# L-Scofano/SEEME

Hardware: AMD Instinct MI355X
Metric: sampled seqs/sec (T=196, 50 DDIM steps) (higher is better)
Workload: dtype f32 accumulate (fp16 denoiser weights, fp16 VAE MFMA operands); 1 GPU; config_mld_egobody interactee-only: VAE encode -> 50-step DDIM -> VAE decode, B=32/GPU, T=196, nfeats=132, random-init recipe weights; batch_per_gpu=32, seq_len=196, ddim_steps=50, parallelism=dp1 (independent shards, no collective on the data path)

## Files before the change

### include/seeme_hip.h

```cpp
#ifndef SEEME_HIP_H
#define SEEME_HIP_H

#include <stddef.h>
#include <stdint.h>

#ifdef __cplusplus
extern "C" {
#endif

#define SEEME_D 256
#define SEEME_NLAYERS 5

enum { SEEME_ACT_NONE = 0, SEEME_ACT_RELU = 1, SEEME_ACT_GELU = 2, SEEME_ACT_SILU = 3 };
enum { SEEME_SCHED_NONE = 0, SEEME_SCHED_DDIM = 1, SEEME_SCHED_DDPM = 2 };

int seeme_version(void);
const char* seeme_last_error(void);

#define SEEME_LINEAR_MAX_K 1008
typedef struct {
    const float* A;  int lda;
    const float* A2; int lda2;
    int K1;
    const float* W;  int ldw;
    const float* bias;
    const float* res; int ldr;
    const float* ln_w; const float* ln_b;
    const float* pre_ln_w; const float* pre_ln_b;
    float* Y; int ldy;
    int M, N, K;
    int pre_act;
    int act;
    float eps;
} SeemeLinearArgs;
int seeme_linear(const SeemeLinearArgs* args, void* stream);

typedef struct {
    const float *in_w, *in_b;
    const float *out_w, *out_b;
    const float *l1_w, *l1_b;
    const float *l2_w, *l2_b;
    const float *n1_w, *n1_b, *n2_w, *n2_b;
    const float *ca_in_w, *ca_in_b;
    const float *ca_out_w, *ca_out_b;
    const float *n3_w, *n3_b;
} SeemeXfLayer;

typedef struct {
    SeemeXfLayer layer[SEEME_NLAYERS];
    const float *skip_w[2], *skip_b[2];
    const float *norm_w, *norm_b;
} SeemeSkipStack;

typedef struct { const uint16_t *in_w, *out_w, *l1_w, *l2_w; } SeemeXfLayerH;
typedef struct {
    SeemeXfLayerH enc[SEEME_NLAYERS], dec[SEEME_NLAYERS];
    const uint16_t *enc_skip[2], *dec_skip[2];
    const uint16_t *emb_w, *fin_w, *ca_fold_w;
    const void* dec_pro; int dec_pro_T;
} SeemeVaeWeightsH;

typedef struct {
    int nfeats;
    int ff;
    const float* token;
    const float* pe_enc;
    const float* pe_dec;
    const float* emb_w; int emb_ldw;
    const float* emb_b;
    const float* fin_w;
    const float* fin_b;
    SeemeSkipStack enc, dec;
    const float* ca_fold_w;
    const float* ca_fold_b;
    const SeemeVaeWeightsH* h16;
} SeemeVaeWeights;

size_t seeme_vae_workspace_bytes(int B, int T);

int seeme_vae_encode(const SeemeVaeWeights* w, const float* features, const int32_t* lengths,
                     int B, int T, float* mu, float* logvar, void* workspace, size_t ws_bytes, void* stream);

int seeme_vae_decode(const SeemeVaeWeights* w, const float* z, const int32_t* lengths,
                     int B, int T, float* feats, void* workspace, size_t ws_bytes, void* stream);

size_t seeme_vae_dec_prologue_bytes(int T);
int seeme_vae_dec_prologue_h16(const SeemeVaeWeights* w, int T, void* buf, size_t bytes, void* stream);

typedef struct {
    const void*  wg;   int wdtype;
    const float* vp;
    const int64_t* layout;
    int nhead;
    int ff_sa;
    int ff;
    const float* kv_cat_w; const float* kv_cat_b;
    const float* style_cat_w; const float* style_cat_b;
    const float* time_w1; const float* time_b1; const float* time_w2; const float* time_b2;
    const float* ca_kv_w[SEEME_NLAYERS]; const float* ca_kv_b[SEEME_NLAYERS];
    const float* ca_tn_w[SEEME_NLAYERS]; const float* ca_tn_b[SEEME_NLAYERS];
    const float* ca_fold_w; const float* ca_fold_b;
    const float* ln_ones; const float* ln_zeros;
    int sa_fold;
    const float* ca_pn_w; const float* ca_pn_b;
    const float* ca_po_w; const float* ca_po_b;
} SeemeDenoiserWeights;

#define SEEME_TROW 7680
#define SEEME_CROW 5120

size_t seeme_denoiser_workspace_bytes(int n_rows, int B, int N);

int seeme_denoiser_time_tables(const SeemeDenoiserWeights* w, const float* tfeat, int n_rows,
                               float* ttab, void* workspace, size_t ws_bytes, void* stream);

int seeme_denoiser_cond_tables(const SeemeDenoiserWeights* w, const float* cond, int Bc, int N,
                               float* ctab, void* workspace, size_t ws_bytes, void* stream);

int seeme_denoiser_ca_tables(const SeemeDenoiserWeights* w, const float* ctab, const float* ttab, const int32_t* trow,
                             int trow_per_sample, int n_trow, int Bc, float* catab,
                             void* workspace, size_t ws_bytes, void* stream);

typedef struct {
    int B;
    int N;
    int steps;
    int sched;
    int cfg;
    float guidance_scale;
    const float* latents;
    const float* ctab;
    const float* ttab;
    const int32_t* trow;
    int trow_per_sample;
    const float* coef;
    const float* noise;
    float* out;
    const float* catab;
    float* save;
    int force_query;
    const unsigned char* drop;
    float drop_scale;
    int xcds;
} SeemeSampleArgs;
#define SEEME_DEN_DROP_BYTES 10960

int seeme_denoiser_sample(const SeemeDenoiserWeights* w, const SeemeSampleArgs* a, void* stream);

typedef struct {
    const void*  wgc;  int wdtype;
    const float* vpc;
    int C;
    int placement;
    int flags;
    void* xchg; size_t xchg_bytes;
    int query;
    int samples;
} SeemeDenCluster;
size_t seeme_den_cluster_xchg_bytes(int B, int C);
size_t seeme_den_cluster_ms_xchg_bytes(int B, int C, int samples);
int seeme_den_cluster_layout(int C, int wdtype, int query, int64_t* out, int cap);
int seeme_denoiser_sample_cluster(const SeemeDenoiserWeights* w, const SeemeDenCluster* cl, const SeemeSampleArgs* a, void* stream);

int seeme_den_train_layout(int64_t* out, int cap);
int seeme_den_train_pack(const float* const* mats, float* img_f, float* img_b, const float* const* vec_src,
                         const int* vec_n, const int64_t* vec_dst, int n_vec, float* vp, void* stream);
int seeme_denoiser_backward(const SeemeDenoiserWeights* w, const void* img_bwd, int B, int N, const float* save,
                            const float* ctab, const float* ttab, const int32_t* trow, const float* dout,
                            float* gout, float* dctab, float* dttab, void* stream);
int seeme_denoiser_backward_drop(const SeemeDenoiserWeights* w, const void* img_bwd, int B, int N, const float* save,
                                 const float* ctab, const float* ttab, const int32_t* trow, const float* dout,
                                 float* gout, float* dctab, float* dttab, const unsigned char* drop, float drop_scale, int xcds, void* stream);

int seeme_den_layout(int ff_sa, int ff, int64_t* out, int cap);

typedef struct {
    int V;
    const float* v_template;
    const float* blend_w;
    const float* lbs_weights;
    const float* J_template;
    const float* J_shapedirs;
    const int32_t* parents;
    const float* ex_template;
    const float* ex_shapedirs;
    const float* ex_posedirs;
    const float* ex_weights;
} SeemeSmplModel;

size_t seeme_smpl_workspace_bytes(int M);

int seeme_smpl_lbs(const SeemeSmplModel* m, const float* betas, const float* pose, int pose_is_rotmat,
                   const float* transl, int M, float* joints, float* vertices,
                   void* workspace, size_t ws_bytes, void* stream);

int seeme_smpl_joints_backward(const SeemeSmplModel* m, const float* betas, const float* pose, const float* djoints, int dj_stride,
                               float* dpose, float* dtransl, int M, void* stream);

int seeme_smpl_joints_rot6d(const SeemeSmplModel* m, const float* betas, const float* r6, int order, const float* transl, int M,
                            float* joints, void* stream);
int seeme_smpl_joints_rot6d_backward(const SeemeSmplModel* m, const float* betas, const float* r6, int order, const float* djoints,
                                     int dj_stride, float* dr6, float* dtransl, int M, void* stream);

enum { SEEME_GEO_AA_TO_QUAT = 0, SEEME_GEO_AA_TO_ROTMAT = 1, SEEME_GEO_QUAT_TO_ROTMAT = 2,
       SEEME_GEO_ROT6D_PROHMR = 3, SEEME_GEO_ROT6D_DIFFUSION = 4 };
int seeme_geometry(int op, const float* in, float* out, int M, void* stream);
int seeme_renorm(const float* x, const float* mean, const float* stdv, float* y, long rows, int F, void* stream);

typedef struct {
    int out_dim;
    const float* pos_w; const float* pos_b;
    const float* fc0_w[4]; const float* fc0_b[4];
    const float* fc1_w[4]; const float* fc1_b[4];
    const float* sc_w[4];
    const float* fcc_w; const float* fcc_b;
} SeemePointnetWeights;
size_t seeme_pointnet_workspace_bytes(int B, int P);
int seeme_pointnet_encode(const SeemePointnetWeights* w, const float* points, int B, int P, float* out,
                          void* workspace, size_t ws_bytes, void* stream);

typedef struct {
    const uint16_t* posf;
    const uint16_t* stream[4];
    const uint16_t* sc3f;
} SeemePointnetBf16;
size_t seeme_pointnet_bf16_workspace_bytes(int B, int P);
int seeme_pointnet_encode_bf16(const SeemePointnetWeights* w, const SeemePointnetBf16* wb, const float* points,
                               int B, int P, float* out, void* workspace, size_t ws_bytes, void* stream);

int seeme_den_wgrad(const float* gout, int ldg, int B, const void* tiles, int n_tiles, float* out, void* stream);
int seeme_den_vecgrad(const float* gout, int ldg, int B, const int64_t* idx, int n, float* out, int dx0_col, float* dpe_row0,
                      void* stream);

int seeme_adamw_step(const void* chunks, int n_chunks, void* const* params, const void* const* grads, void* const* exp_avg,
                     void* const* exp_avg_sq, double lr, double beta1, double beta2, double eps, double weight_decay,
                     double step, void* stream);

int seeme_adamw_step_dev(const void* chunks, int n_chunks, void* const* params, const void* const* grads, void* const* exp_avg,
                         void* const* exp_avg_sq, const float* step_lr, double beta1, double beta2, double eps,
                         double weight_decay, void* stream);

typedef struct {
    const void* chunks;
    int n_chunks;
    void* const* params;
    const void* const* grads;
    void* const* exp_avg;
    void* const* exp_avg_sq;
    void* const* ema;
    const float* step_lr;
    double lr, step;
    double beta1, beta2, eps, weight_decay;
    double ema_decay;
    int ema_warmup;
    const float* grad_scale;
} SeemeAdamWEx;
int seeme_adamw_step_ex(const SeemeAdamWEx* a, void* stream);
int seeme_adamw_ex_bytes(void);

size_t seeme_grad_norm_workspace_bytes(int n_chunks);
int seeme_grad_norm(const void* chunks, int n_chunks, const void* const* grads, double max_norm, float* out ,
                    void* ws, size_t ws_bytes, void* stream);

typedef struct {
    int B, N;
    const float* dist;
    int dist_rows;
    const float* eps_z;
    const float* eps_c;
    int slot_c;
    float* cond;
    const float* noise;
    const int64_t* timesteps;
    const float* acp;
    const float* freq;
    int flip_sin_to_cos;
    float* latents;
    float* noisy;
    float* tfeat;
} SeemeGlueRows;
int seeme_glue_rows(const SeemeGlueRows* a, void* stream);
int seeme_glue_ln(const float* x, float* xhat, float* rstd, int M, void* stream);

typedef struct {
    const float* a[10];
    const float* b[10];
    int seg_len[10];
    long a_ks[10];
    long b_ks[10];
    int nseg;
    long a_rs, b_cs;
    float* c;
    long ldc;
    int M, N;
    int a_pro;
    const float* a_p0;
    const float* a_p1;
    int b_pro;
    const float* b_p0;
    const float* b_p1;
    const float* bias;
    int epi;
    const float* e0;
    long e_ld;
    int accumulate;
    float* colsum;
    int tile0, tiles_n;
    int nbatch;
    long a_bstride, b_bstride, c_bstride;
    float alpha;
// ... 178 lines not shown
```

### seeme_amd/_lib.py

```python
from __future__ import annotations

import ctypes as C
import os
from typing import Optional

_HERE = os.path.dirname(os.path.abspath(__file__))
LIB_PATH = os.environ.get("SEEME_HIP_LIB") or os.path.join(_HERE, "libseeme_hip.so")

NLAYERS = 5
TROW = 7680
CROW = 5120
ACT_NONE, ACT_RELU, ACT_GELU, ACT_SILU = 0, 1, 2, 3
SCHED_NONE, SCHED_DDIM, SCHED_DDPM = 0, 1, 2

fp = C.c_void_p


class SeemeError(RuntimeError):
    pass


class LinearArgs(C.Structure):
    _fields_ = [("A", fp), ("lda", C.c_int), ("A2", fp), ("lda2", C.c_int), ("K1", C.c_int),
                ("W", fp), ("ldw", C.c_int), ("bias", fp), ("res", fp), ("ldr", C.c_int),
                ("ln_w", fp), ("ln_b", fp), ("pre_ln_w", fp), ("pre_ln_b", fp),
                ("Y", fp), ("ldy", C.c_int), ("M", C.c_int), ("N", C.c_int), ("K", C.c_int),
                ("pre_act", C.c_int), ("act", C.c_int), ("eps", C.c_float)]


class XfLayer(C.Structure):
    _fields_ = [(n, fp) for n in ("in_w", "in_b", "out_w", "out_b", "l1_w", "l1_b", "l2_w", "l2_b",
                                  "n1_w", "n1_b", "n2_w", "n2_b",
                                  "ca_in_w", "ca_in_b", "ca_out_w", "ca_out_b", "n3_w", "n3_b")]


class SkipStack(C.Structure):
    _fields_ = [("layer", XfLayer * NLAYERS), ("skip_w", fp * 2), ("skip_b", fp * 2),
                ("norm_w", fp), ("norm_b", fp)]


class XfLayerH(C.Structure):
    _fields_ = [(n, fp) for n in ("in_w", "out_w", "l1_w", "l2_w")]


class VaeWeightsH(C.Structure):
    _fields_ = [("enc", XfLayerH * NLAYERS), ("dec", XfLayerH * NLAYERS), ("enc_skip", fp * 2), ("dec_skip", fp * 2),
                ("emb_w", fp), ("fin_w", fp), ("ca_fold_w", fp), ("dec_pro", fp), ("dec_pro_T", C.c_int)]


def pack_mfma16(W, dtype):
    import torch
    N, K = W.shape
    Np, Kp = (N + 15) // 16 * 16, (K + 31) // 32 * 32
    Wz = torch.zeros(Np, Kp, device=W.device, dtype=dtype)
    Wz[:N, :K] = W.detach().to(dtype)
    return Wz.view(Np // 16, 16, Kp // 32, 4, 8).permute(0, 2, 3, 1, 4).contiguous()


class VaeWeights(C.Structure):
    _fields_ = [("nfeats", C.c_int), ("ff", C.c_int), ("token", fp), ("pe_enc", fp), ("pe_dec", fp),
                ("emb_w", fp), ("emb_ldw", C.c_int), ("emb_b", fp), ("fin_w", fp), ("fin_b", fp),
                ("enc", SkipStack), ("dec", SkipStack), ("ca_fold_w", fp), ("ca_fold_b", fp), ("h16", fp)]


class DenoiserWeights(C.Structure):
    _fields_ = [("wg", fp), ("wdtype", C.c_int), ("vp", fp), ("layout", fp), ("nhead", C.c_int), ("ff_sa", C.c_int),
                ("ff", C.c_int), ("kv_cat_w", fp), ("kv_cat_b", fp), ("style_cat_w", fp), ("style_cat_b", fp),
                ("time_w1", fp), ("time_b1", fp), ("time_w2", fp), ("time_b2", fp),
                ("ca_kv_w", fp * NLAYERS), ("ca_kv_b", fp * NLAYERS),
                ("ca_tn_w", fp * NLAYERS), ("ca_tn_b", fp * NLAYERS),
                ("ca_fold_w", fp), ("ca_fold_b", fp), ("ln_ones", fp), ("ln_zeros", fp), ("sa_fold", C.c_int),
                ("ca_pn_w", fp), ("ca_pn_b", fp), ("ca_po_w", fp), ("ca_po_b", fp)]


class SampleArgs(C.Structure):
    _fields_ = [("B", C.c_int), ("N", C.c_int), ("steps", C.c_int), ("sched", C.c_int), ("cfg", C.c_int),
                ("guidance_scale", C.c_float), ("latents", fp), ("ctab", fp), ("ttab", fp), ("trow", fp),
                ("trow_per_sample", C.c_int), ("coef", fp), ("noise", fp), ("out", fp), ("catab", fp), ("save", fp), ("force_query", C.c_int), ("drop", fp), ("drop_scale", C.c_float), ("xcds", C.c_int)]


class DenCluster(C.Structure):
    _fields_ = [("wgc", fp), ("wdtype", C.c_int), ("vpc", fp), ("C", C.c_int), ("placement", C.c_int), ("flags", C.c_int),
                ("xchg", fp), ("xchg_bytes", C.c_size_t), ("query", C.c_int), ("samples", C.c_int)]


class SmplModel(C.Structure):
    _fields_ = [("V", C.c_int), ("v_template", fp), ("blend_w", fp), ("lbs_weights", fp), ("J_template", fp),
                ("J_shapedirs", fp), ("parents", fp), ("ex_template", fp), ("ex_shapedirs", fp),
                ("ex_posedirs", fp), ("ex_weights", fp)]


class PointnetWeights(C.Structure):
    _fields_ = [("out_dim", C.c_int), ("pos_w", fp), ("pos_b", fp), ("fc0_w", fp * 4), ("fc0_b", fp * 4),
                ("fc1_w", fp * 4), ("fc1_b", fp * 4), ("sc_w", fp * 4), ("fcc_w", fp), ("fcc_b", fp)]


class PointnetBf16(C.Structure):
    _fields_ = [("posf", fp), ("stream", fp * 4), ("sc3f", fp)]


class GlueRows(C.Structure):
    _fields_ = [("B", C.c_int), ("N", C.c_int), ("dist", fp), ("dist_rows", C.c_int), ("eps_z", fp), ("eps_c", fp),
                ("slot_c", C.c_int), ("cond", fp), ("noise", fp), ("timesteps", fp), ("acp", fp), ("freq", fp),
                ("flip_sin_to_cos", C.c_int), ("latents", fp), ("noisy", fp), ("tfeat", fp)]


class GemmProblem(C.Structure):
    _fields_ = [("a", fp * 10), ("b", fp * 10), ("seg_len", C.c_int * 10), ("a_ks", C.c_long * 10),
                ("b_ks", C.c_long * 10), ("nseg", C.c_int), ("a_rs", C.c_long), ("b_cs", C.c_long), ("c", fp), ("ldc", C.c_long),
                ("M", C.c_int), ("N", C.c_int), ("a_pro", C.c_int), ("a_p0", fp), ("a_p1", fp), ("b_pro", C.c_int),
                ("b_p0", fp), ("b_p1", fp), ("bias", fp), ("epi", C.c_int), ("e0", fp), ("e_ld", C.c_long),
                ("accumulate", C.c_int), ("colsum", fp), ("tile0", C.c_int), ("tiles_n", C.c_int), ("nbatch", C.c_int),
                ("a_bstride", C.c_long), ("b_bstride", C.c_long), ("c_bstride", C.c_long), ("alpha", C.c_float), ("addend", fp),
                ("add_ld", C.c_long)]


class VtLn(C.Structure):
    _fields_ = [("sub", fp), ("res", fp), ("gamma", fp), ("beta", fp), ("y", fp), ("xhat", fp), ("rstd", fp), ("M", C.c_long),
                ("sub_seq_rows", C.c_int), ("eps", C.c_float)]


class VtLnBwd(C.Structure):
    _fields_ = [("dy", fp), ("xhat", fp), ("rstd", fp), ("gamma", fp), ("dpre", fp), ("dgamma", fp), ("dbeta", fp), ("M", C.c_long),
                ("accumulate", C.c_int), ("dy2", fp)]


class GlueMid(C.Structure):
    _fields_ = [("M", C.c_int), ("B", C.c_int), ("dxl", fp), ("dcs", fp), ("xhat", fp), ("rstd", fp), ("tn_w", fp * 5),
                ("g_tn_w", fp * 5), ("g_tn_b", fp * 5), ("dcond", fp), ("dea", fp), ("deb", fp), ("emb", fp), ("demb", fp)]


class AdamWEx(C.Structure):
    _fields_ = [("chunks", fp), ("n_chunks", C.c_int), ("params", fp), ("grads", fp), ("exp_avg", fp), ("exp_avg_sq", fp),
                ("ema", fp), ("step_lr", fp), ("lr", C.c_double), ("step", C.c_double), ("beta1", C.c_double), ("beta2", C.c_double),
                ("eps", C.c_double), ("weight_decay", C.c_double), ("ema_decay", C.c_double), ("ema_warmup", C.c_int),
                ("grad_scale", fp)]


RESNET_FP32, RESNET_BF16 = 0, 1
IMG_F32_NCHW, IMG_U8_NHWC = 0, 1
RESNET50_NCONV = 53


class Conv(C.Structure):
    _fields_ = [("weight", fp), ("weight_bf16", fp), ("bias", fp), ("cin", C.c_int), ("cout", C.c_int), ("k", C.c_int),
                ("stride", C.c_int)]


class Resnet50(C.Structure):
    _fields_ = [("precision", C.c_int), ("conv", Conv * RESNET50_NCONV), ("tap", fp * 5)]


class RenderScene(C.Structure):
    _fields_ = [("verts", fp), ("faces", fp), ("points", fp), ("cams", fp)] + \
               [(n, C.c_int) for n in ("F", "NV", "NF", "P", "FC", "H", "W", "point_size")] + \
               [(n, C.c_float) for n in ("fx", "fy", "cx", "cy", "znear")]


class FlowHead(C.Structure):
    _fields_ = [(n, fp) for n in ("ctx_w", "ctx_b", "id_w", "lin_w", "bn_s", "bn_o", "res_b", "fin_w", "fin_b", "lu_w", "act_s",
                                  "act_o", "fc_w", "fc_b")] + [("id_parity", C.c_int), ("log_const", C.c_float)]


GEO_AA_TO_QUAT, GEO_AA_TO_ROTMAT, GEO_QUAT_TO_ROTMAT, GEO_ROT6D_PROHMR, GEO_ROT6D_DIFFUSION = range(5)

_SIGNATURES = {
    "seeme_smpl_joints_backward": (C.c_int, [C.POINTER(SmplModel), fp, fp, fp, C.c_int, fp, fp, C.c_int, fp]),
    "seeme_smpl_joints_rot6d": (C.c_int, [C.POINTER(SmplModel), fp, fp, C.c_int, fp, C.c_int, fp, fp]),
    "seeme_smpl_joints_rot6d_backward": (C.c_int, [C.POINTER(SmplModel), fp, fp, C.c_int, fp, C.c_int, fp, fp, C.c_int, fp]),
    "seeme_vt_add_ln": (C.c_int, [C.POINTER(VtLn), fp]),
    "seeme_vt_ln_bwd": (C.c_int, [C.POINTER(VtLnBwd), fp]),
    "seeme_vt_softmax_fwd": (C.c_int, [fp, fp, C.c_int, C.c_int, C.c_int, C.c_float, fp]),
    "seeme_vt_softmax_bwd": (C.c_int, [fp, fp, C.c_long, C.c_int, C.c_float, fp]),
    "seeme_vt_gelu": (C.c_int, [fp, fp, fp, C.c_long, fp]),
    "seeme_vt_seq_sum": (C.c_int, [fp, fp, C.c_int, C.c_int, C.c_int, fp, C.c_float, fp]),
    "seeme_vt_dropout": (C.c_int, [fp, fp, C.c_float, fp, C.c_long, fp]),
    "seeme_vt_cross_rows": (C.c_int, [fp, fp, fp, fp, C.c_float, C.c_int, C.c_int, fp, fp]),
    "seeme_den_vecgrad": (C.c_int, [fp, C.c_int, C.c_int, fp, C.c_int, fp, C.c_int, fp, fp]),
    "seeme_glue_rows": (C.c_int, [C.POINTER(GlueRows), fp]),
    "seeme_glue_ln": (C.c_int, [fp, fp, fp, C.c_int, fp]),
    "seeme_glue_mid": (C.c_int, [C.POINTER(GlueMid), fp]),
    "seeme_grouped_gemm": (C.c_int, [fp, C.c_int, C.c_int, fp]),
    "seeme_gemm_problem_bytes": (C.c_int, []),
    "seeme_wgrad128": (C.c_int, [fp, C.c_long, fp, C.c_long, C.c_int, C.c_int, C.c_int, fp, C.c_long, fp, fp]),
    "seeme_gemm128": (C.c_int, [fp, C.c_long, fp, C.c_long, C.c_int, fp, C.c_long, C.c_int, C.c_int, C.c_int, fp, fp, C.c_long, fp]),
    "seeme_version": (C.c_int, []),
    "seeme_last_error": (C.c_char_p, []),
    "seeme_linear": (C.c_int, [C.POINTER(LinearArgs), fp]),
    "seeme_vae_workspace_bytes": (C.c_size_t, [C.c_int, C.c_int]),
    "seeme_vae_encode": (C.c_int, [C.POINTER(VaeWeights), fp, fp, C.c_int, C.c_int, fp, fp, fp, C.c_size_t, fp]),
    "seeme_vae_decode": (C.c_int, [C.POINTER(VaeWeights), fp, fp, C.c_int, C.c_int, fp, fp, C.c_size_t, fp]),
    "seeme_vae_dec_prologue_bytes": (C.c_size_t, [C.c_int]),
    "seeme_vae_dec_prologue_h16": (C.c_int, [C.POINTER(VaeWeights), C.c_int, fp, C.c_size_t, fp]),
    "seeme_denoiser_workspace_bytes": (C.c_size_t, [C.c_int, C.c_int, C.c_int]),
    "seeme_denoiser_time_tables": (C.c_int, [C.POINTER(DenoiserWeights), fp, C.c_int, fp, fp, C.c_size_t, fp]),
    "seeme_denoiser_cond_tables": (C.c_int, [C.POINTER(DenoiserWeights), fp, C.c_int, C.c_int, fp, fp, C.c_size_t, fp]),
    "seeme_denoiser_ca_tables": (C.c_int, [C.POINTER(DenoiserWeights), fp, fp, fp, C.c_int, C.c_int, C.c_int, fp, fp, C.c_size_t, fp]),
    "seeme_denoiser_sample": (C.c_int, [C.POINTER(DenoiserWeights), C.POINTER(SampleArgs), fp]),
    "seeme_denoiser_sample_cluster": (C.c_int, [C.POINTER(DenoiserWeights), C.POINTER(DenCluster), C.POINTER(SampleArgs), fp]),
    "seeme_den_cluster_xchg_bytes": (C.c_size_t, [C.c_int, C.c_int]),
    "seeme_den_cluster_ms_xchg_bytes": (C.c_size_t, [C.c_int, C.c_int, C.c_int]),
    "seeme_den_cluster_layout": (C.c_int, [C.c_int, C.c_int, C.c_int, C.POINTER(C.c_int64), C.c_int]),
    "seeme_den_train_layout": (C.c_int, [C.POINTER(C.c_int64), C.c_int]),
    "seeme_den_train_pack": (C.c_int, [fp, fp, fp, fp, C.POINTER(C.c_int), C.POINTER(C.c_int64), C.c_int, fp, fp]),
    "seeme_denoiser_backward": (C.c_int, [C.POINTER(DenoiserWeights), fp, C.c_int, C.c_int, fp, fp, fp, fp, fp, fp, fp, fp, fp]),
    "seeme_denoiser_backward_drop": (C.c_int, [C.POINTER(DenoiserWeights), fp, C.c_int, C.c_int, fp, fp, fp, fp, fp, fp, fp, fp, fp, C.c_float, C.c_int, fp]),
    "seeme_den_layout": (C.c_int, [C.c_int, C.c_int, C.POINTER(C.c_int64), C.c_int]),
    "seeme_den_wgrad": (C.c_int, [fp, C.c_int, C.c_int, fp, C.c_int, fp, fp]),
    "seeme_adamw_step": (C.c_int, [fp, C.c_int, fp, fp, fp, fp, C.c_double, C.c_double, C.c_double, C.c_double, C.c_double,
                                   C.c_double, fp]),
    "seeme_adamw_step_dev": (C.c_int, [fp, C.c_int, fp, fp, fp, fp, fp, C.c_double, C.c_double, C.c_double, C.c_double, fp]),
    "seeme_adamw_step_ex": (C.c_int, [C.POINTER(AdamWEx), fp]),
    "seeme_adamw_ex_bytes": (C.c_int, []),
    "seeme_grad_norm_workspace_bytes": (C.c_size_t, [C.c_int]),
    "seeme_grad_norm": (C.c_int, [fp, C.c_int, fp, C.c_double, fp, fp, C.c_size_t, fp]),
    "seeme_geometry": (C.c_int, [C.c_int, fp, fp, C.c_int, fp]),
    "seeme_renorm": (C.c_int, [fp, fp, fp, fp, C.c_long, C.c_int, fp]),
    "seeme_pointnet_workspace_bytes": (C.c_size_t, [C.c_int, C.c_int]),
    "seeme_pointnet_encode": (C.c_int, [C.POINTER(PointnetWeights), fp, C.c_int, C.c_int, fp, fp, C.c_size_t, fp]),
    "seeme_pointnet_bf16_workspace_bytes": (C.c_size_t, [C.c_int, C.c_int]),
    "seeme_pointnet_encode_bf16": (C.c_int, [C.POINTER(PointnetWeights), C.POINTER(PointnetBf16), fp, C.c_int, C.c_int, fp, fp,
                                             C.c_size_t, fp]),
    "seeme_smpl_workspace_bytes": (C.c_size_t, [C.c_int]),
    "seeme_smpl_lbs": (C.c_int, [C.POINTER(SmplModel), fp, fp, C.c_int, fp, C.c_int, fp, fp, fp, C.c_size_t, fp]),
    "seeme_hyp_metrics_workspace_bytes": (C.c_size_t, [C.c_int, C.c_int, C.c_int]),
    "seeme_hyp_metrics": (C.c_int, [fp, fp, fp, C.c_int, C.c_int, C.c_int, fp, fp, fp, C.c_size_t, fp]),
    "seeme_hyp_pairdist_workspace_bytes": (C.c_size_t, [C.c_int, C.c_int, C.c_int]),
    "seeme_hyp_pairdist": (C.c_int, [fp, fp, C.c_int, C.c_int, C.c_int, fp, fp, fp, C.c_size_t, fp]),
    "seeme_social_metrics_workspace_bytes": (C.c_size_t, [C.c_int, C.c_int, C.c_int]),
    "seeme_social_metrics": (C.c_int, [fp, fp, fp, fp, fp, fp, fp, C.c_int, C.c_int, C.c_int, fp, fp, fp, C.c_size_t, fp]),
    "seeme_overlap_cost_workspace_bytes": (C.c_size_t, [C.c_int, C.c_int, C.c_int, C.c_int]),
    "seeme_overlap_cost": (C.c_int, [fp, C.c_int, C.c_int, C.c_int, C.c_int, fp, fp, C.c_size_t, fp]),
    "seeme_path_select_workspace_bytes": (C.c_size_t, [C.c_int, C.c_int]),
    "seeme_path_select": (C.c_int, [fp, fp, C.c_int, C.c_int, fp, fp, fp, fp, C.c_size_t, fp]),
    "seeme_stitch_windows": (C.c_int, [fp, C.c_int, C.c_int, C.c_int, C.c_int, C.c_int, C.c_int, fp, fp]),
    "seeme_scene_views_workspace_bytes": (C.c_size_t, [C.c_int, C.c_int, C.c_int]),
    "seeme_scene_views": (C.c_int, [fp, fp, C.c_int, C.c_int, C.c_int, fp, fp, fp, fp, C.c_size_t, fp]),
    "seeme_crop_patches": (C.c_int, [fp, C.c_int, C.c_int, C.c_int, fp, fp, C.c_int, C.c_int, fp, fp]),
    "seeme_render_workspace_bytes": (C.c_size_t, [C.c_int, C.c_int, C.c_int, C.c_int]),
    "seeme_render": (C.c_int, [C.POINTER(RenderScene), fp, fp, fp, fp, C.c_size_t, fp]),
    "seeme_render_shade": (C.c_int, [C.POINTER(RenderScene), fp, fp, fp, C.c_int, fp, C.c_uint32, fp, fp]),
    "seeme_pa_mpjpe_frames": (C.c_int, [fp, fp, fp, C.c_int, fp, fp]),
    "seeme_mesh_v2v_frames": (C.c_int, [fp, fp, fp, fp, fp, C.c_int, C.c_int, fp, fp]),
    "seeme_scene_min_dist2_workspace_bytes": (C.c_size_t, [C.c_int, C.c_int, C.c_int, C.c_int]),
    "seeme_scene_min_dist2": (C.c_int, [fp, fp, fp, C.c_int, C.c_int, C.c_int, C.c_int, fp, fp, C.c_size_t, fp]),
    "seeme_scene_inside_count_workspace_bytes": (C.c_size_t, [C.c_int, C.c_int, C.c_int, C.c_int]),
    "seeme_scene_inside_count": (C.c_int, [fp, fp, C.c_int, fp, fp, C.c_int, C.c_int, C.c_int, C.c_int, fp, fp, C.c_size_t, fp]),
    "seeme_mesh_winding": (C.c_int, [fp, fp, C.c_int, fp, fp, C.c_int, C.c_int, C.c_int, C.c_int, fp, fp]),
    "seeme_flow_head_workspace_bytes": (C.c_size_t, [C.c_int, C.c_int]),
    "seeme_flow_head": (C.c_int, [C.POINTER(FlowHead), fp, fp, C.c_int, C.c_int, fp, fp, fp, fp, fp, fp, C.c_size_t, fp]),
    "seeme_resnet50_workspace_bytes": (C.c_size_t, [C.c_int, C.c_int]),
    "seeme_resnet50_encode": (C.c_int, [C.POINTER(Resnet50), fp, C.c_int, C.c_int, fp, fp, C.c_size_t, fp]),
    "seeme_resnet_conv": (C.c_int, [C.POINTER(Conv), C.c_int, fp, C.c_int, C.c_int, C.c_int, fp, C.c_int, fp, fp]),
    "seeme_resnet_stem_pack": (C.c_int, [fp, C.c_int, C.c_int, C.c_int, C.c_int, C.c_int, fp, fp]),
    "seeme_resnet_maxpool": (C.c_int, [C.c_int, fp, C.c_int, C.c_int, C.c_int, C.c_int, fp, fp]),
}

_lib: Optional[C.CDLL] = None


def lib() -> C.CDLL:
    global _lib
    if _lib is None:
        if not os.path.exists(LIB_PATH):
            raise SeemeError(
                f"{LIB_PATH} is missing: build it with `python -c 'import __graft_entry__ as g; g.build()'` "
                "or seeme_amd/csrc/build.sh.  There is no CPU / PyTorch fallback for this path.")
        try:
            l = C.CDLL(LIB_PATH)
        except OSError as e:
            raise SeemeError(f"cannot load {LIB_PATH}: {e}") from e
        for name, (res, args) in _SIGNATURES.items():
            f = getattr(l, name)
            f.restype = res
            f.argtypes = args
        _lib = l
    return _lib


def exported_symbols():
    return sorted(_SIGNATURES)


def check(rc: int, what: str = ""):
    if rc != 0:
        msg = lib().seeme_last_error().decode("utf-8", "replace")
        raise SeemeError(f"{what or 'seeme_hip'} failed (rc={rc}): {msg}")


def call(name: str, *args):
    check(getattr(lib(), name)(*args), name)


class Workspace:

    def __init__(self, per_stream: bool):
        self.per_stream = per_stream
        self._held = {}

    def get(self, need: int, device):
        import torch
        device = torch.device(device)
        if device.type == "cuda" and device.index is None:
            device = torch.device("cuda", torch.cuda.current_device())
        key = device
        if self.per_stream and device.type == "cuda":
            key = (device, torch.cuda.current_stream(device).cuda_stream)
        ws = self._held.get(key)
        if ws is None or ws.numel() < max(need, 16):
            ws = None
            self._held.pop(key, None)
            ws = self._held[key] = torch.empty(max(int(need), 16), dtype=torch.uint8, device=device)
        return ws

    def cached(self) -> list:
        return list(self._held.values())

    def fill_(self, byte: int):
        for ws in self._held.values():
            ws.fill_(byte)


def default_xcds(chains: int, want="auto") -> int:
    e = os.environ.get("SEEME_DEN_XCDS")
    if e is not None:
        want = int(e)
    if want == "auto":
        want = (chains + 15) // 16
    return min(8, max(1, int(want)))


def ptr(t) -> int:
    return 0 if t is None else t.data_ptr()


def current_stream() -> int:
    import torch
    return torch.cuda.current_stream().cuda_stream


def require_cuda(t, name: str):
    import torch
    if not isinstance(t, torch.Tensor) or not t.is_cuda:
        raise SeemeError(f"{name} must be a tensor on the ROCm device (cuda:N); this path has no CPU fallback")
    if t.dtype != torch.float32:
        raise SeemeError(f"{name} must be float32, got {t.dtype}")
```

### seeme_amd/csrc/den_cluster.inc.hip

```cpp

#define DCL_MAGIC_EPOCH 0x7fffffffu
#define DCL_SPIN_LIMIT (1u << 22)

typedef __attribute__((address_space(1))) unsigned long long dcl_gu64;

template <typename WT> struct ClW {
    static constexpr int KL = WT::MFMA ? 32 : 16;
    static constexpr int UL = 256 / KL;
    static constexpr int RU = WT::MFMA ? 4 : 2;
    static constexpr unsigned UNIT_BYTES = 8u * UL * 1024u;
};
template <int C, bool Q = false> struct ClG {
    static constexpr int S = 256 / C;
    static constexpr int NB = 1024 / C;
    static constexpr int TA = S / 32;
    static constexpr int TB = 8 / C;
    static constexpr int U_A = 0, U_AS = TA, U_B = 2 * TA, U_C = U_B + TB;
    static constexpr int U_G = U_C + TB, U_H = U_G + 1;
    static constexpr int U_D = Q ? U_H + 2 : U_C + TB, U_E = U_D + 1, U_F = U_E + 1, NU_REAL = U_F + 2;
    static constexpr int NU = (NU_REAL + 3) / 4 * 4;
    static constexpr int SC = Q ? 8 : 4;
    static constexpr int X1_G = 2 * S + SC;
    static constexpr int G_BOOT = 0, G_X1 = 16, G_X2 = G_X1 + C * X1_G, G_X3 = G_X2 + C * 256, G_TOTAL = G_X3 + (Q ? C * 8 : 0);
    static constexpr int EPL = Q ? 3 : 2;
// ... 935 lines not shown
                __syncthreads(); DEN_DBG(0);
            }

            if constexpr (Q) nxt.load(3, wave, lane, vp, Ln, tt_next, ln, A, b, c, ca_next, ca_R);
            if constexpr (!Q && !WIN) cl_refills<WT, C, Q, G::U_C + C_INL>(ring, wave, voff, wg, bc, bn, skip, nskip, std::make_integer_sequence<int, G::TB - C_INL>{});
            if constexpr (GRP) {
                clg_issue<0>(gr, gvoff, wg, bn + (unsigned)G::U_A * W::UNIT_BYTES, true, nskip || w4 < 2);
            } else {
                f32x4 acc[1];
                cl_zero<1>(acc);
                cl_units<WT, C, Q, G::U_D, 1, 1, 0, 0, (WIN ? 0 : 1)>(ring, xa, acc, true, wave, voff, wg, bc, bn, skip, nskip, std::make_integer_sequence<int, 1>{});
                if (lane < 16) {
                    const int j = wave * 16 + col;
                    cl_put1<WT>(XH, j, fast_gelu(cl_out<WT>(acc[0]) + v_f1b[j]));
                }
            }
            if constexpr (Q) nxt.store(lane, STG + (cur ^ 1) * stg_sz);
            __syncthreads(); DEN_DBG(0);
            if constexpr (GRP) {
                f32x4 acc[2][2];
                uint4 fr[4];
                clg_frags<4>(fr, xh);
                __builtin_amdgcn_sched_barrier(0);
                cl_zero<2>(acc[0]); cl_zero<2>(acc[1]);
                clg_consume<WT, 2, 4, 0>(gr.r[1], fr, acc);
                cl_pin<2>(acc[0]); cl_pin<2>(acc[1]);
                PART[(2 * (w4 + 4 * (lane >> 5)) + ((lane >> 4) & 1)) * 16 + col] = clg_out<WT, 2>(acc, lane);
            } else {
                f32x4 acc[2];
                cl_zero<2>(acc);
                cl_units<WT, C, Q, G::U_E, 1, 2, 0, 0, (WIN ? 0 : 1)>(ring, xh, acc, true, wave, voff, wg, bc, bn, skip, nskip, std::make_integer_sequence<int, 1>{});
                if (lane < 32) PART[(2 * wave + (lane >> 4)) * 16 + col] = (lane & 16) ? cl_out<WT>(acc[1]) : cl_out<WT>(acc[0]);
            }
            __syncthreads(); DEN_DBG(0);
            if (epi) {
                if constexpr (WIN) {
                    cl_issue_seq<WT, C, Q>(ring, wave, voff, wg, bc, bn, skip, nskip, typename SCH::W3{});
                    if (lane == 0) cl_flag_set(FLG + 3, e2);
                }
                const float4 y2 = f4_add(ld4(PART + 4 * lane), ld4(v_f2b + 4 * lane));
                const float4 hh = f4_adaln(wave_ln(y2, v_fsnw, v_fsnb, lane), ld4(TFS + 4 * lane), ld4(TFS + 256 + 4 * lane));
                put_x<WT, 1>(XB, 0, 0, lane, f4_silu(hh));
            } else if constexpr (WIN) {
                cl_flag_wait(FLG + 3, e2);
                cl_issue_seq<WT, C, Q>(ring, wave, voff, wg, bc, bn, skip, nskip, typename SCH::W3{});
            }
            __syncthreads(); DEN_DBG(0);
            if constexpr (Q) nxt.load(4, wave, lane, vp, Ln, tt_next, ln, A, b, c, ca_next, ca_R);
            if constexpr (WIN) __builtin_amdgcn_sched_barrier(0);
            if constexpr (GRP) {
                clg_issue<1>(gr, gvoff, wg, bn + (unsigned)G::U_AS * W::UNIT_BYTES, nskip, nskip);
            } else {
                f32x4 acc[2];
                cl_zero<2>(acc);
                cl_units<WT, C, Q, G::U_F, 2, 2, 0, 0, (WIN ? 0 : 2)>(ring, xb, acc, true, wave, voff, wg, bc, bn, skip, nskip, std::make_integer_sequence<int, 2>{});
                if constexpr (WIN) cl_issue_seq<WT, C, Q>(ring, wave, voff, wg, bc, bn, skip, nskip, typename SCH::AF{});
                if (lane < 32) {
                    const int n = (2 * wave + (lane >> 4)) * 16 + col;
                    const float xn = RES[n] + ((lane & 16) ? cl_out<WT>(acc[1]) : cl_out<WT>(acc[0])) + v_fo_b[n];
                    RES[n] = xn;
                    cl_put1<WT>(XA, n, xn);
                    if (l < 2) cl_put1<WT>(SKF + 512 * l, n, xn);
                }
            }
            if constexpr (Q) nxt.store(lane, STG + (cur ^ 1) * stg_sz);
            if constexpr (!WIN) cl_refills<WT, C, Q, G::NU_REAL>(ring, wave, voff, wg, bc, bn, skip, nskip, std::make_integer_sequence<int, G::NU - G::NU_REAL>{});
            __syncthreads(); DEN_DBG(0);
            if (l + 1 < SEEME_DEN_NL) {
                if (epi && !nskip) xr = ld4(RES + 4 * lane);
            } else {
                if (epi) {
                    float4 e = wave_ln(ld4(RES + 4 * lane), CONSTV + 256, CONSTV + 512, lane);
                    if (A.sched == SEEME_SCHED_NONE) {
                        st4(KEEP + 4 * lane, e);
                    } else {
                        float c0, c1, c2, c3, c4, c5, clip, ptype;
                        float4 nz = make_float4(0.f, 0.f, 0.f, 0.f);
                        if constexpr (GRP) {
                            const float4 k0 = ld4(COEF), k1 = ld4(COEF + 4);
                            const auto sc = [](float v) { return __uint_as_float(__builtin_amdgcn_readfirstlane(__float_as_uint(v))); };
                            c0 = sc(k0.x); c1 = sc(k0.y); c2 = sc(k0.z); c3 = sc(k0.w); c4 = sc(k1.x); c5 = sc(k1.y); clip = sc(k1.z); ptype = sc(k1.w);
                            if (A.noise != nullptr) nz = ld4(NZ + 4 * lane);
                        } else {
                            const CF32 cf = coef_c + (size_t)step * 8;
                            c0 = cf[0]; c1 = cf[1]; c2 = cf[2]; c3 = cf[3]; c4 = cf[4]; c5 = cf[5]; clip = cf[6]; ptype = cf[7];
                            if (A.noise != nullptr) nz = ld4(A.noise + ((size_t)step * A.B + b) * 256 + 4 * lane);
                        }
                        const float4 lat = ld4(KEEP + 4 * lane);
                        const float xs[4] = {lat.x, lat.y, lat.z, lat.w}, es4[4] = {e.x, e.y, e.z, e.w}, ns[4] = {nz.x, nz.y, nz.z, nz.w};
                        float o[4];
                        if constexpr (GRP) {
#pragma unroll
                            for (int i = 0; i < 4; ++i) o[i] = cl_sched_elem(i == 3, xs[i], es4[i], ns[i], c0, c1, c2, c3, c4, c5, clip, ptype);
                        } else {
#pragma unroll
                            for (int i = 0; i < 4; ++i) {
                                float x0, ep;
                                if (ptype == 0.f) { ep = es4[i]; x0 = (xs[i] - c1 * ep) / c0; }
                                else              { x0 = es4[i]; ep = (xs[i] - c0 * x0) / c1; }
                                if (clip != 0.f) x0 = fminf(fmaxf(x0, -1.f), 1.f);
                                o[i] = c2 * x0 + c3 * ep + c5 * xs[i] + c4 * ns[i];
                            }
                        }
                        const float4 nl = make_float4(o[0], o[1], o[2], o[3]);
                        st4(KEEP + 4 * lane, nl);
                        xr = f4_add(nl, ld4(CONSTV + 4 * lane));
                        put_x<WT, 1>(XA, 0, 0, lane, xr);
                        st4(RES + 4 * lane, xr);
                    }
                }
                __syncthreads(); DEN_DBG(0);
            }
            cur ^= 1;
        }
        row = GRP ? row_nx : row_next;
    }
    DEN_DBG(3);
    if (epi && c == 0) st4(A.out + (size_t)b * 256 + 4 * lane, ld4(KEEP + 4 * lane));
    if constexpr (GRP) {
#pragma unroll
        for (int s = 0; s < 2; ++s) asm volatile("" ::"v"(gr.r[s][0][0].x));
    } else {
#pragma unroll
        for (int s = 0; s < W::RU; ++s) asm volatile("" ::"v"(ring.r[s][0].x));
    }
}

template <int C>
static size_t cl_lds_bytes(int N, bool q, bool grp) {
    typedef ClG<C> G;
    const int stg = q ? 2 * (VP_LAYER + STG_TT + N * 1024) : ClRes<C>::FLOATS;
    const int sch = grp ? 12 + 256 : 0;
    return (size_t)(768 + 256 + stg + 512 + 512 + 2 * (G::NB > 128 ? G::NB : 128) + 1024 + 2 * G::S + 256 + 256 + 4 + sch) * sizeof(float);
}

extern "C" size_t seeme_den_cluster_xchg_bytes(int B, int C) {
    const size_t per = C == 8 ? ClG<8, true>::G_TOTAL : (C == 4 ? ClG<4, true>::G_TOTAL : ClG<2, true>::G_TOTAL);
    const size_t clusters = (size_t)(B + 7) / 8 * 8;
    return DCL_HDR_BYTES + clusters * per * 8;
}
extern "C" int seeme_den_cluster_layout(int C, int wdtype, int query, int64_t* out, int cap) {
    if (cap < 14) return seeme_fail("den_cluster_layout: output too small");
    if (C != 2 && C != 4 && C != 8) return seeme_fail("den_cluster_layout: C must be 2, 4 or 8");
    const int TA = 256 / C / 32, TB = 8 / C;
    const int u_c = 2 * TA + TB, u_g = u_c + TB, u_d = query ? u_g + 3 : u_g;
    const int64_t NU = (u_d + 4 + 3) / 4 * 4, UL = wdtype == 0 ? 16 : 8, UB = 8 * UL * 1024;
    out[0] = NU; out[1] = UB; out[2] = (int64_t)SEEME_DEN_NL * C * NU * UB; out[3] = UL; out[4] = 256 / UL;
    out[5] = 0; out[6] = TA; out[7] = 2 * TA; out[8] = u_c; out[9] = u_d; out[10] = u_d + 1; out[11] = u_d + 2;
    out[12] = query ? u_g : -1; out[13] = query ? u_g + 1 : -1;
    return 0;
}

template <typename WT, int C, bool Q>
static int launch_den_cluster(const ClArgs& ka0, hipStream_t st) {
    ClArgs ka = ka0;
    ka.clusters = (ka.s.B + 7) / 8 * 8;
    const int grid = ka.clusters * C;
    int dev = 0, cus = 0;
    SEEME_HIP(hipGetDevice(&dev));
    SEEME_HIP(hipDeviceGetAttribute(&cus, hipDeviceAttributeMultiprocessorCount, dev));
    if (grid > cus || grid > 256) return seeme_fail("denoiser_sample_cluster: B x C exceeds one workgroup per CU of this device");
    const size_t lds = cl_lds_bytes<C>(Q ? ka.s.N : 1, Q, ClGrp<WT, C, Q>::ON);
    if (lds > 160 * 1024 || lds <= 80 * 1024) return seeme_fail("denoiser_sample_cluster: LDS footprint must force one workgroup per CU");
    SEEME_HIP(hipFuncSetAttribute((const void*)k_den_cluster<WT, C, Q>, hipFuncAttributeMaxDynamicSharedMemorySize, (int)lds));
    SEEME_HIP(hipMemsetAsync(ka.hdr, 0, seeme_den_cluster_xchg_bytes(ka.s.B, C), st));
    hipLaunchKernelGGL((k_den_cluster<WT, C, Q>), dim3(grid), dim3(DEN_THREADS), lds, st, ka);
    return seeme_check_launch("k_den_cluster");
}
template <typename WT>
static int launch_den_cluster_c(const ClArgs& ka, int C, bool q, hipStream_t st) {
    if (C == 8) return q ? launch_den_cluster<WT, 8, true>(ka, st) : launch_den_cluster<WT, 8, false>(ka, st);
    if (C == 4) return q ? launch_den_cluster<WT, 4, true>(ka, st) : launch_den_cluster<WT, 4, false>(ka, st);
    if (C == 2) return q ? launch_den_cluster<WT, 2, true>(ka, st) : launch_den_cluster<WT, 2, false>(ka, st);
    return seeme_fail("denoiser_sample_cluster: C must be 2, 4 or 8");
}

static int den_cluster_ms_dispatch(const SeemeDenoiserWeights* w, const SeemeDenCluster* cl, const SeemeSampleArgs* a, ClArgs& ka, hipStream_t st);

extern "C" int seeme_denoiser_sample_cluster(const SeemeDenoiserWeights* w, const SeemeDenCluster* cl, const SeemeSampleArgs* a, void* stream) {
    if (a->B <= 0) return seeme_fail("denoiser_sample_cluster: B must be > 0");
    if (a->N < 1 || a->N > DCL_MAX_N) return seeme_fail("denoiser_sample_cluster: 1 or 2 condition tokens");
    const bool q = a->N > 1;
    if (!q && (a->catab == nullptr || a->force_query)) return seeme_fail("denoiser_sample_cluster: one condition token needs its ca table");
    if (q != (cl->query != 0)) return seeme_fail("denoiser_sample_cluster: the weight image was packed for the other ca_block variant (SeemeDenCluster.query)");
    if (w->nhead != 1 || !w->sa_fold) return seeme_fail("denoiser_sample_cluster: one attention head (folded out_proj)");
    if (a->cfg || a->save != nullptr) return seeme_fail("denoiser_sample_cluster: no CFG pair, no training forward");
    if (w->ff_sa != FF_SA || w->ff != FF_D) return seeme_fail("denoiser_sample_cluster: built for sa ff 1024 / ffn_dim 128");
    if (a->sched == SEEME_SCHED_NONE && a->steps != 1) return seeme_fail("denoiser_sample_cluster: SCHED_NONE needs steps == 1");
    if (a->steps < 1) return seeme_fail("denoiser_sample_cluster: steps must be >= 1");
    const bool ms = cl->samples > 1;
    if (cl->xchg == nullptr || (!ms && cl->xchg_bytes < seeme_den_cluster_xchg_bytes(a->B, cl->C))) return seeme_fail("denoiser_sample_cluster: exchange buffer too small");
    if (((uintptr_t)cl->xchg & 15) != 0) return seeme_fail("denoiser_sample_cluster: exchange buffer must be 16-byte aligned");
    int64_t lo[14];
    int rc = seeme_den_cluster_layout(cl->C, cl->wdtype, q ? 1 : 0, lo, 14);
    if (rc) return rc;
    ClArgs ka;
    ka.wgc = cl->wgc; ka.wgc_bytes = (unsigned)lo[2]; ka.vp = cl->vpc;
    ka.lay = seeme_make_den_layout(FF_SA, FF_D);
    ka.s = *a;
    ka.hdr = (unsigned*)cl->xchg;
    ka.xg = (unsigned long long*)((char*)cl->xchg + DCL_HDR_BYTES);
    ka.placement = cl->placement; ka.flags = cl->flags; ka.clusters = 0; ka.spc = 1;
    hipStream_t st = (hipStream_t)stream;
    if (ms) return den_cluster_ms_dispatch(w, cl, a, ka, st);
    if (cl->wdtype == 0) return launch_den_cluster_c<WF32>(ka, cl->C, q, st);
    if (cl->wdtype == 1) return launch_den_cluster_c<WBF16>(ka, cl->C, q, st);
    if (cl->wdtype == 2) return launch_den_cluster_c<WF16>(ka, cl->C, q, st);
    return seeme_fail("denoiser_sample_cluster: wdtype must be 0 (fp32), 1 (bf16) or 2 (fp16)");
}
```

### seeme_amd/csrc/den_cluster_ms.inc.hip

```cpp

#ifndef DCLM_POLL_SLEEP
#define DCLM_POLL_SLEEP 8
#endif
#ifndef DCLM_SENTINEL_FROM
#define DCLM_SENTINEL_FROM 5
#endif


template <typename WT, bool NARROW> struct ClmRows {
    static_assert(WT::HALF || !NARROW, "the bf16 split has three parts");
    static constexpr int MS = NARROW ? 8 : 4, SPL = NARROW ? 2 : 1, ROWB = NARROW ? 32 : 64;
};
template <typename WT, int C, bool Q = false, bool NARROW = true> struct ClM {
    typedef ClG<C, Q> G;
    static constexpr int MS = ClmRows<WT, NARROW>::MS;
    static constexpr int SPL = ClmRows<WT, NARROW>::SPL;
    static constexpr int XKB = 1024;
    static constexpr int XBUF = 256 / 32 * XKB / 4;
    static constexpr int XHK = G::NB > 128 ? G::NB : 128;
    static constexpr int XHBUF = XHK / 32 * XKB / 4;
    static constexpr int O_SKIPB = 0, O_INB = G::S , O_N1W = 4 * G::S, O_N1B = O_N1W + 256, O_L2B = O_N1B + 256,
                         O_N2W = O_L2B + 256, O_N2B = O_N2W + 256, O_F1B = O_N2B + 256, O_F2B = O_F1B + FF_D, O_FSNW = O_F2B + 256,
                         O_FSNB = O_FSNW + 256, O_FOB = O_FSNB + 256, O_L1B = O_FOB + 256,
                         O_TK = O_L1B + G::NB , O_TV = O_TK + 256, O_TSC = O_TV + 256, O_TSH = O_TSC + 256,
// ... 556 lines not shown
                    float Lw = lc * wc;
                    if (C >= 2) Lw += dpp_f(Lw, 0);
                    if (C >= 4) Lw += dpp_f(Lw, 1);
                    if (C >= 8) Lw += dpp_f(Lw, 2);
                    const float rL = fast_rcp(Lw);
                    float4 y = make_float4(0.f, 0.f, 0.f, 0.f);
#pragma unroll
                    for (int n = 0; n < N; ++n) {
                        float t = __uint_as_float((n & 1) ? g3[1 + (n >> 1)].z : g3[1 + (n >> 1)].x) * wc;
                        if (C >= 2) t += dpp_f(t, 0);
                        if (C >= 4) t += dpp_f(t, 1);
                        if (C >= 8) t += dpp_f(t, 2);
                        y = f4_fma(t * rL, cav[n], y);
                    }
                    const float4 hh = f4_adaln(wave_ln(y, VP + M::O_CSNW, VP + M::O_CSNB, lane), ld4(VP + M::O_CSC + 4 * lane), ld4(VP + M::O_CSH + 4 * lane));
                    clm_put4<WT, NARROW>(XB, es, lane, f4_silu(hh));
                } else {
                    clm_wait_published(FLG + 2, pub3);
                    cl_issue_seq<WT, C, Q>(ring, wave, voff, wg, bc, bn, skip, nskip, typename SCH::WXA{});
                    cl_flag_wait(FLG + 3, e3);
                    cl_issue_seq<WT, C, Q>(ring, wave, voff, wg, bc, bn, skip, nskip, typename SCH::WXB{});
                }
                __syncthreads(); DEN_DBG(0);
                nxt.load(2, wave, lane, vp, Ln, tt_next, ln, A, b0, nact, c);
                {
                    f32x4 acc[2];
                    cl_zero<2>(acc);
                    cl_units<WT, C, Q, G::U_H, 2, 2, 0, 0, 0>(ring, xb, acc, true, wave, voff, wg, bc, bn, skip, nskip, std::make_integer_sequence<int, 2>{});
#pragma unroll
                    for (int tt = 0; tt < 2; ++tt) {
                        const int n = (2 * wave + tt) * 16 + col;
                        const float bo = VP[M::O_CAOB + n];
#pragma unroll
                        for (int j = 0; j < SPL; ++j) {
                            const int sj = g2 + j;
                            if (sj < nact) {
                                const float x3 = RES[sj * 256 + n] + clm_out<WT, NARROW>(acc[tt], j) + bo;
                                RES[sj * 256 + n] = x3;
                                clm_put1<WT, NARROW>(XA, sj, n, x3);
                            }
                        }
                    }
                }
                nxt.store(lane, STGN);
                __syncthreads(); DEN_DBG(0);
            }

            nxt.load(Q ? 3 : 1, wave, lane, vp, Ln, tt_next, ln, A, b0, nact, c);
            {
                f32x4 acc[1];
                cl_zero<1>(acc);
                cl_units<WT, C, Q, G::U_D, 1, 1, 0, 0, 0>(ring, xa, acc, true, wave, voff, wg, bc, bn, skip, nskip, std::make_integer_sequence<int, 1>{});
                const int jh = wave * 16 + col;
                const float bh = VP[M::O_F1B + jh];
#pragma unroll
                for (int j = 0; j < SPL; ++j)
                    if (g2 + j < nact) clm_put1<WT, NARROW>(XH, g2 + j, jh, fast_gelu(clm_out<WT, NARROW>(acc[0], j) + bh));
            }
            nxt.store(lane, STGN);
            __syncthreads(); DEN_DBG(0);
            {
                f32x4 acc[2];
                cl_zero<2>(acc);
                cl_units<WT, C, Q, G::U_E, 1, 2, 0, 0, 0>(ring, xh, acc, true, wave, voff, wg, bc, bn, skip, nskip, std::make_integer_sequence<int, 1>{});
#pragma unroll
                for (int tt = 0; tt < 2; ++tt)
#pragma unroll
                    for (int j = 0; j < SPL; ++j)
                        if (g2 + j < nact) PART[(g2 + j) * 256 + (2 * wave + tt) * 16 + col] = clm_out<WT, NARROW>(acc[tt], j);
            }
            __syncthreads(); DEN_DBG(0);
            cl_issue_seq<WT, C, Q>(ring, wave, voff, wg, bc, bn, skip, nskip, typename SCH::W3{});
            if (epi) {
                const float4 y2 = f4_add(ld4(PART + es * 256 + 4 * lane), ld4(VP + M::O_F2B + 4 * lane));
                const float4 hh = f4_adaln(wave_ln(y2, VP + M::O_FSNW, VP + M::O_FSNB, lane), ld4(VP + M::O_TSC + 4 * lane), ld4(VP + M::O_TSH + 4 * lane));
                clm_put4<WT, NARROW>(XB, es, lane, f4_silu(hh));
            }
            __syncthreads(); DEN_DBG(0);
            nxt.load(Q ? 4 : 2, wave, lane, vp, Ln, tt_next, ln, A, b0, nact, c);
            {
                f32x4 acc[2];
                cl_zero<2>(acc);
                cl_units<WT, C, Q, G::U_F, 2, 2, 0, 0, 0>(ring, xb, acc, true, wave, voff, wg, bc, bn, skip, nskip, std::make_integer_sequence<int, 2>{});
                cl_issue_seq<WT, C, Q>(ring, wave, voff, wg, bc, bn, skip, nskip, typename SCH::AF{});
#pragma unroll
                for (int tt = 0; tt < 2; ++tt) {
                    const int n = (2 * wave + tt) * 16 + col;
                    const float bo = VP[M::O_FOB + n];
#pragma unroll
                    for (int j = 0; j < SPL; ++j) {
                        const int sj = g2 + j;
                        if (sj < nact) {
                            const float xn = RES[sj * 256 + n] + clm_out<WT, NARROW>(acc[tt], j) + bo;
                            RES[sj * 256 + n] = xn;
                            clm_put1<WT, NARROW>(XA, sj, n, xn);
                            if (l < 2) clm_put1<WT, NARROW>(SKF + M::XBUF * l, sj, n, xn);
                        }
                    }
                }
            }
            nxt.store(lane, STGN);
            __syncthreads(); DEN_DBG(0);
            if (l + 1 < SEEME_DEN_NL) {
                if (epi && !nskip) xr = ld4(RES + es * 256 + 4 * lane);
            } else {
                if (epi) {
                    float4 e = wave_ln(ld4(RES + es * 256 + 4 * lane), CONSTV + 256, CONSTV + 512, lane);
                    if (A.sched == SEEME_SCHED_NONE) {
                        st4(KEEP + es * 256 + 4 * lane, e);
                    } else {
                        const CF32 cf = coef_c + (size_t)step * 8;
                        const float c0 = cf[0], c1 = cf[1], c2 = cf[2], c3 = cf[3], c4 = cf[4], c5 = cf[5], clip = cf[6], ptype = cf[7];
                        float4 nz = make_float4(0.f, 0.f, 0.f, 0.f);
                        if (A.noise != nullptr) nz = ld4(A.noise + ((size_t)step * A.B + bs) * 256 + 4 * lane);
                        const float4 lat = ld4(KEEP + es * 256 + 4 * lane);
                        const float xs[4] = {lat.x, lat.y, lat.z, lat.w}, es4[4] = {e.x, e.y, e.z, e.w}, ns[4] = {nz.x, nz.y, nz.z, nz.w};
                        float o[4];
#pragma unroll
                        for (int i = 0; i < 4; ++i) {
                            float x0, ep;
                            if (ptype == 0.f) { ep = es4[i]; x0 = (xs[i] - c1 * ep) / c0; }
                            else              { x0 = es4[i]; ep = (xs[i] - c0 * x0) / c1; }
                            if (clip != 0.f) x0 = fminf(fmaxf(x0, -1.f), 1.f);
                            o[i] = c2 * x0 + c3 * ep + c5 * xs[i] + c4 * ns[i];
                        }
                        const float4 nl = make_float4(o[0], o[1], o[2], o[3]);
                        st4(KEEP + es * 256 + 4 * lane, nl);
                        xr = f4_add(nl, ld4(CONSTV + 4 * lane));
                        clm_put4<WT, NARROW>(XA, es, lane, xr);
                        st4(RES + es * 256 + 4 * lane, xr);
                    }
                }
                __syncthreads(); DEN_DBG(0);
            }
            cur ^= 1;
        }
        row = row_next;
    }
    DEN_DBG(3);
    if (epi && c == 0) st4(A.out + (size_t)bs * 256 + 4 * lane, ld4(KEEP + es * 256 + 4 * lane));
#pragma unroll
    for (int s = 0; s < W::RU; ++s) asm volatile("" ::"v"(ring.r[s][0].x));
}

static int clm_clusters(int B, int spc) { return ((B + spc - 1) / spc + 7) / 8 * 8; }

extern "C" size_t seeme_den_cluster_ms_xchg_bytes(int B, int C, int spc) {
    if (spc < 1 || spc > 8 || (C != 4 && C != 8)) return 0;
    const size_t per = C == 8 ? ClG<8, true>::G_TOTAL : ClG<4, true>::G_TOTAL;
    return DCL_HDR_BYTES + (size_t)clm_clusters(B, spc) * 8 * per * 8;
}

template <typename WT, int C, bool Q, bool NARROW>
static int launch_den_cluster_ms(const ClArgs& ka0, hipStream_t st) {
    ClArgs ka = ka0;
    ka.clusters = clm_clusters(ka.s.B, ka.spc);
    const int grid = ka.clusters * C;
    int dev = 0, cus = 0;
    SEEME_HIP(hipGetDevice(&dev));
    SEEME_HIP(hipDeviceGetAttribute(&cus, hipDeviceAttributeMultiprocessorCount, dev));
    if (grid > cus || grid > 256) return seeme_fail("denoiser_sample_cluster: clusters x C exceeds one workgroup per CU of this device");
    if (ka0.spc > ClM<WT, C, Q, NARROW>::MS) return seeme_fail("denoiser_sample_cluster: at most 8 (fp16) / 4 (bf16) samples per cluster");
    const size_t lds = (size_t)ClM<WT, C, Q, NARROW>::LDS_FLOATS * sizeof(float);
    if (lds > 160 * 1024 || lds <= 80 * 1024) return seeme_fail("denoiser_sample_cluster: LDS footprint must force one workgroup per CU");
    SEEME_HIP(hipFuncSetAttribute((const void*)k_den_cluster_ms<WT, C, Q, NARROW>, hipFuncAttributeMaxDynamicSharedMemorySize, (int)lds));
    SEEME_HIP(hipMemsetAsync(ka.hdr, 0, seeme_den_cluster_ms_xchg_bytes(ka.s.B, C, ka.spc), st));
    hipLaunchKernelGGL((k_den_cluster_ms<WT, C, Q, NARROW>), dim3(grid), dim3(DEN_THREADS), lds, st, ka);
    return seeme_check_launch("k_den_cluster_ms");
}

static int den_cluster_ms_dispatch(const SeemeDenoiserWeights* w, const SeemeDenCluster* cl, const SeemeSampleArgs* a, ClArgs& ka, hipStream_t st) {
    if (cl->wdtype != 2 && cl->wdtype != 1) return seeme_fail("denoiser_sample_cluster: several samples per cluster need a 16-bit weight image");
    if (cl->C != 4 && cl->C != 8) return seeme_fail("denoiser_sample_cluster: several samples per cluster need C = 4 or 8");
    if (cl->samples > 8) return seeme_fail("denoiser_sample_cluster: at most 8 samples per cluster");
    if (a->N != 1 && a->N != 2) return seeme_fail("denoiser_sample_cluster: several samples per cluster need one or two condition tokens");
    if (a->trow_per_sample) return seeme_fail("denoiser_sample_cluster: several samples per cluster share the step's table row");
    if (cl->xchg_bytes < seeme_den_cluster_ms_xchg_bytes(a->B, cl->C, cl->samples)) return seeme_fail("denoiser_sample_cluster: exchange buffer too small");
    ka.spc = cl->samples;
    if (cl->wdtype == 1) {
        if (cl->C != 4) return seeme_fail("denoiser_sample_cluster: the bf16 image takes several samples per cluster at C = 4 only");
        return a->N == 2 ? launch_den_cluster_ms<WBF16, 4, true, false>(ka, st) : launch_den_cluster_ms<WBF16, 4, false, false>(ka, st);
    }
    if (cl->C == 4 && cl->samples <= 4)
        return a->N == 2 ? launch_den_cluster_ms<WF16, 4, true, false>(ka, st) : launch_den_cluster_ms<WF16, 4, false, false>(ka, st);
    if (a->N == 2) return cl->C == 8 ? launch_den_cluster_ms<WF16, 8, true, true>(ka, st) : launch_den_cluster_ms<WF16, 4, true, true>(ka, st);
    return cl->C == 8 ? launch_den_cluster_ms<WF16, 8, false, true>(ka, st) : launch_den_cluster_ms<WF16, 4, false, true>(ka, st);
}
```

### seeme_amd/csrc/den_kernels.hip

```cpp
#include <atomic>
#include "common.hpp"
#include "api_util.hpp"
#include "den_layout.h"
#include "lds_ring.hpp"
#include "den_train.h"
#include <utility>

#define DEN_THREADS 512
#define SEEME_DEN_PAIR_ABOVE 256
#define DEN_MAXTOK 6
#define DEN_R 4
#define DEN_CH 8

struct WF32 { typedef float T; static constexpr int KV = 4; static constexpr bool HALF = false, MFMA = false; static constexpr int PARTS = 1; };
struct WBF16 { typedef uint16_t T; static constexpr int KV = 8; static constexpr bool HALF = false, MFMA = true; static constexpr int PARTS = 3; };
struct WF16 { typedef uint16_t T; static constexpr int KV = 8; static constexpr bool HALF = true, MFMA = true; static constexpr int PARTS = 2; };
#define DEN_F16_LO_SCALE 2048.f

typedef float f2 __attribute__((ext_vector_type(2)));
typedef unsigned int u32x4 __attribute__((ext_vector_type(4)));
typedef float f32x4 __attribute__((ext_vector_type(4)));
typedef _Float16 h16x8 __attribute__((ext_vector_type(8)));
typedef __bf16 bf16x8 __attribute__((ext_vector_type(8)));

// ... 790 lines not shown
                    xr = f4_add(nl, ld4(CONSTV + 4 * lane));
                    put_x<WT, MS>(XB, es, 0, lane, xr);
                }
                __syncthreads(); DEN_DBG(0);
            }
            cur ^= 1;
        }
        row = row_next;
    }
    DEN_DBG(3);
    if (epi && (es == 0 || (!A.cfg && MS * b + es < A.B))) st4(A.out + (size_t)bl * 256 + 4 * lane, ld4(keep));
#pragma unroll
    for (int s = 0; s < DEN_R; ++s) asm volatile("" ::"v"(ring.r[s][0].x));
}

static size_t den_lds_bytes(int MS, int N, bool mfma) {
    return (size_t)(768 + MS * 768 + 2 * (VP_LAYER + STG_TT + MS * N * 1024 + (N > 1 ? 0 : MS * 256)) + XB_FLOATS(mfma, MS) + (mfma ? MS * 1024 : 4 * MS * 768)) * sizeof(float);
}

static int den_xcd_grid(int chains, int want, int* xcds) {
    int k = (want >= 1 && want <= 7) ? want : 8;
    if (chains > 32 * k) k = 8;
    *xcds = k;
    return k < 8 ? (chains + k - 1) / k * 8 : chains;
}
template <typename WT, int MS, int V>
static int launch_den(const DenKArgs& ka, hipStream_t st) {
    const int chains = (MS == 2 && !ka.s.cfg) ? (ka.s.B + 1) / 2 : ka.s.B;
    const size_t lds = den_lds_bytes(MS, ka.s.N, WT::MFMA);
    if (lds > 160 * 1024) return seeme_fail("denoiser_sample: LDS budget exceeded");
    SEEME_HIP(hipFuncSetAttribute((const void*)k_den_sample<WT, MS, V>, hipFuncAttributeMaxDynamicSharedMemorySize, (int)lds));
    DenKArgs k2 = ka;
    k2.chains = chains;
    const int grid = den_xcd_grid(chains, ka.s.xcds, &k2.xcds);
    hipLaunchKernelGGL((k_den_sample<WT, MS, V>), dim3(grid), dim3(DEN_THREADS), lds, st, k2);
    return seeme_check_launch("k_den_sample");
}
template <typename WT, int MS>
static int launch_den_ms(const DenKArgs& ka, bool fold, hipStream_t st) {
    const bool caq = ka.s.N > 1 || ka.s.force_query;
    if (caq) return fold ? launch_den<WT, MS, V_CAQ | V_FOLD>(ka, st) : launch_den<WT, MS, V_CAQ>(ka, st);
    return fold ? launch_den<WT, MS, V_FOLD>(ka, st) : launch_den<WT, MS, 0>(ka, st);
}
template <typename WT>
static int launch_den_wt(const DenKArgs& ka, bool fold, hipStream_t st) {
    const bool pair = ka.s.cfg || (ka.s.B > SEEME_DEN_PAIR_ABOVE && !ka.s.trow_per_sample);
    return pair ? launch_den_ms<WT, 2>(ka, fold, st) : launch_den_ms<WT, 1>(ka, fold, st);
}

extern "C" int seeme_denoiser_sample(const SeemeDenoiserWeights* w, const SeemeSampleArgs* a, void* stream) {
    if (a->B <= 0) return seeme_fail("denoiser_sample: B must be > 0");
    if (a->N < 1 || a->N > DEN_MAXTOK - 2) return seeme_fail("denoiser_sample: 1 <= N <= 4 condition tokens");
    if (w->nhead != 1 && w->nhead != 2 && w->nhead != 4) return seeme_fail("denoiser_sample: nhead must be 1, 2 or 4");
    if (w->ff_sa != FF_SA || w->ff != FF_D) return seeme_fail("denoiser_sample: built for sa ff 1024 / ffn_dim 128 (all reference configs)");
    if (w->layout == nullptr) return seeme_fail("denoiser_sample: layout table missing");
    if (a->sched == SEEME_SCHED_NONE && a->steps != 1) return seeme_fail("denoiser_sample: SCHED_NONE needs steps == 1");
    if (a->steps < 1) return seeme_fail("denoiser_sample: steps must be >= 1");
    if (a->save != nullptr && (a->steps != 1 || a->cfg || w->sa_fold || w->wdtype != 0 || !(a->N > 1 || a->force_query) || !a->trow_per_sample))
        return seeme_fail("denoiser_sample: save needs one step, no CFG, the unfolded fp32 image, the query GEMV and per-sample rows");
    DenKArgs ka;
    ka.wg = w->wg; ka.vp = w->vp; ka.lay = seeme_make_den_layout(FF_SA, FF_D);
    ka.wg_bytes = (int)(ka.lay.wg_total * (w->wdtype == 0 ? 4 : 2));
    ka.nhead = w->nhead; ka.s = *a;
    hipStream_t st = (hipStream_t)stream;
    const bool fold = w->sa_fold != 0;
    if (fold && w->nhead != 1) return seeme_fail("denoiser_sample: sa_fold needs nhead == 1");
    if (a->N == 1 && a->catab == nullptr && !a->force_query) return seeme_fail("denoiser_sample: N == 1 needs the ca table (seeme_denoiser_ca_tables)");
    if (w->wdtype == 0) return launch_den_wt<WF32>(ka, fold, st);
    if (w->wdtype == 1) return launch_den_wt<WBF16>(ka, fold, st);
    if (w->wdtype == 2) return launch_den_wt<WF16>(ka, fold, st);
    return seeme_fail("denoiser_sample: wdtype must be 0 (fp32), 1 (bf16) or 2 (fp16)");
}

extern "C" int seeme_den_layout(int ff_sa, int ff, int64_t* out, int cap) {
    if (cap < SEEME_DEN_LAYOUT_FIELDS) return seeme_fail("seeme_den_layout: output too small");
    const DenLayout lay = seeme_make_den_layout(ff_sa, ff);
    int k = 0;
    for (int l = 0; l < SEEME_DEN_NL; ++l) {
        const int64_t* f = reinterpret_cast<const int64_t*>(&lay.L[l]);
        for (int i = 0; i < SEEME_DEN_LAYER_FIELDS; ++i) out[k++] = f[i];
    }
    out[k++] = lay.pe0; out[k++] = lay.fnw; out[k++] = lay.fnb; out[k++] = lay.wg_total; out[k++] = lay.vp_total;
    return 0;
}

extern "C" size_t seeme_denoiser_workspace_bytes(int n_rows, int B, int N) {
    (void)B; (void)N;
    return (size_t)n_rows * 256 * 2 * sizeof(float) + 256;
}

extern "C" int seeme_denoiser_time_tables(const SeemeDenoiserWeights* w, const float* tfeat, int n_rows,
                                          float* ttab, void* workspace, size_t ws_bytes, void* stream) {
    hipStream_t st = (hipStream_t)stream;
    if (ws_bytes < seeme_denoiser_workspace_bytes(n_rows, 0, 0)) return seeme_fail("time_tables: workspace too small");
    float* t1 = (float*)workspace;
    float* temb = t1 + (size_t)n_rows * 256;
    int rc;
    if ((rc = seeme_linear_simple(st, tfeat, 256, w->time_w1, 256, w->time_b1, t1, 256, n_rows, 256, 256, SEEME_ACT_SILU, 0, nullptr, nullptr))) return rc;
    if ((rc = seeme_linear_simple(st, t1, 256, w->time_w2, 256, w->time_b2, temb, 256, n_rows, 256, 256, 0, 0, nullptr, nullptr))) return rc;
    if ((rc = seeme_linear_simple(st, temb, 256, w->kv_cat_w, 256, w->kv_cat_b, ttab, SEEME_TROW, n_rows, 2560, 256, 0, 0, nullptr, nullptr))) return rc;
    return seeme_linear_simple(st, temb, 256, w->style_cat_w, 256, w->style_cat_b, ttab + 2560, SEEME_TROW, n_rows, 5120, 256, 0, SEEME_ACT_SILU, nullptr, nullptr);
}

extern "C" int seeme_denoiser_cond_tables(const SeemeDenoiserWeights* w, const float* cond, int Bc, int N,
                                          float* ctab, void* workspace, size_t ws_bytes, void* stream) {
    (void)workspace; (void)ws_bytes;
    hipStream_t st = (hipStream_t)stream;
    const int M = Bc * N;
    if (w->ca_fold_w == nullptr) return seeme_fail("cond_tables: folded key/value weights missing");
    LinearKArgs ka{};
    ka.a.A = cond; ka.a.lda = 256; ka.a.K1 = 256; ka.a.K = 256; ka.a.W = w->kv_cat_w; ka.a.ldw = 256; ka.a.bias = w->kv_cat_b;
    ka.a.Y = ctab; ka.a.ldy = SEEME_CROW; ka.a.M = M; ka.a.N = 2560; ka.a.eps = 1e-5f;
    ka.a.pre_ln_w = w->ln_ones; ka.a.pre_ln_b = w->ln_zeros;
    ka.nz = 2; ka.zs_a = 0; ka.zs_w = (long)(w->ca_fold_w - w->kv_cat_w); ka.zs_b = (long)(w->ca_fold_b - w->kv_cat_b); ka.zs_y = 2560;
    ka.zs_ln = 0; ka.pre_ln_zmin = 1;
    return seeme_launch_linear(ka, st);
}

__global__ __launch_bounds__(256) void k_ca_rows(const float* __restrict__ ctab, const float* __restrict__ ttab,
                                                 const int32_t* __restrict__ trow, int per_sample, int n_trow, int R, int rows,
                                                 const float* __restrict__ nw, const float* __restrict__ nb, float* __restrict__ H) {
    const int lane = threadIdx.x & 63, l = blockIdx.y;
    const int r0 = blockIdx.x * 4 + (threadIdx.x >> 6);
    if (r0 >= rows) return;
    const int bc = r0 / R, r = r0 - bc * R;
    const int row = per_sample ? trow[bc % n_trow] : trow[r];
    const float4 v = ld4(ctab + (size_t)bc * SEEME_CROW + 2560 + l * 512 + 256 + 4 * lane);
    const float4 hn = wave_ln(v, nw + l * 256, nb + l * 256, lane);
    const float* tt = ttab + (size_t)row * SEEME_TROW + 2560 + l * 1024;
    st4(H + ((size_t)l * rows + r0) * 256 + 4 * lane, f4_silu(f4_adaln(hn, ld4(tt + 4 * lane), ld4(tt + 256 + 4 * lane))));
}

extern "C" int seeme_denoiser_ca_tables(const SeemeDenoiserWeights* w, const float* ctab, const float* ttab, const int32_t* trow,
                                        int trow_per_sample, int n_trow, int Bc, float* catab,
                                        void* workspace, size_t ws_bytes, void* stream) {
    hipStream_t st = (hipStream_t)stream;
    if (Bc <= 0 || n_trow <= 0) return seeme_fail("ca_tables: empty batch / row list");
    const int R = trow_per_sample ? 1 : n_trow;
    const int rows = Bc * R;
    if (ws_bytes < (size_t)SEEME_DEN_NL * rows * 256 * sizeof(float)) return seeme_fail("ca_tables: workspace too small");
    if (w->ca_pn_w == nullptr || w->ca_po_w == nullptr) return seeme_fail("ca_tables: proj_out weights missing");
    float* H = (float*)workspace;
    hipLaunchKernelGGL(k_ca_rows, dim3((rows + 3) / 4, SEEME_DEN_NL), dim3(256), 0, st, ctab, ttab, trow, trow_per_sample, n_trow, R, rows,
                       w->ca_pn_w, w->ca_pn_b, H);
    int rc = seeme_check_launch("k_ca_rows");
    if (rc) return rc;
    LinearKArgs ka{};
    ka.a.A = H; ka.a.lda = 256; ka.a.K1 = 256; ka.a.W = w->ca_po_w; ka.a.ldw = 256; ka.a.bias = w->ca_po_b;
    ka.a.Y = catab; ka.a.ldy = SEEME_DEN_NL * 256; ka.a.M = rows; ka.a.N = 256; ka.a.K = 256; ka.a.eps = 1e-5f;
    ka.nz = SEEME_DEN_NL; ka.zs_a = (long)rows * 256; ka.zs_w = 256 * 256; ka.zs_b = 256; ka.zs_y = 256;
    return seeme_launch_linear(ka, st);
}

#ifdef DEN_DBG_TIMES
extern "C" int seeme_debug_den_times(unsigned long long* host, int n) {
    SEEME_HIP(hipMemcpyFromSymbol(host, HIP_SYMBOL(den_dbg_times), sizeof(unsigned long long) * (size_t)(n < 512 ? n : 512)));
    return 0;
}
#endif

#include "den_train.inc.hip"
#include "den_cluster.inc.hip"
#include "den_cluster_ms.inc.hip"
```

### seeme_amd/csrc/vae_h16.hip

```cpp
#include "common.hpp"
#include "api_util.hpp"

typedef _Float16 h16x8 __attribute__((ext_vector_type(8)));
#define HPAD 16

__device__ __forceinline__ unsigned short f2h(float x) { return __builtin_bit_cast(unsigned short, (_Float16)x); }
__device__ __forceinline__ float h_exp(float x) { return __builtin_amdgcn_exp2f(x * 1.44269504088896340736f); }
__device__ __forceinline__ float h_gelu(float x) {
    const float z = fabsf(x) * 0.70710678118654752440f;
    const float t = __builtin_amdgcn_rcpf(fmaf(0.3275911f, z, 1.f));
    const float poly = t * fmaf(t, fmaf(t, fmaf(t, fmaf(t, 1.061405429f, -1.453152027f), 1.421413741f), -0.284496736f), 0.254829592f);
    return 0.5f * x * (1.f + copysignf(1.f - poly * h_exp(-z * z), x));
}
__device__ __forceinline__ float h_act(float v, int act) { return act == SEEME_ACT_GELU ? h_gelu(v) : act_apply(v, act); }

#ifdef H16_DBG_TIMES
__device__ unsigned long long h16_dbg_times[32];
#ifndef H16_DBG_KERNEL
#define H16_DBG_KERNEL 1
#endif
#define H16_DBG(k, i) do { if (H16_DBG_KERNEL == (k) && blockIdx.x == 3 && blockIdx.y == ((k) == 1 ? 5 : 0) && threadIdx.x == 0) h16_dbg_times[i] = __builtin_readcyclecounter(); } while (0)
extern "C" int seeme_debug_h16_times(unsigned long long* host, int n) {
    SEEME_HIP(hipMemcpyFromSymbol(host, HIP_SYMBOL(h16_dbg_times), sizeof(unsigned long long) * (size_t)(n < 32 ? n : 32)));
    return 0;
// ... 953 lines not shown
            for (int rr = 0; rr < RW; ++rr) x1[rr] = make_float4(x1[rr].x + cv.x, x1[rr].y + cv.y, x1[rr].z + cv.z, x1[rr].w + cv.w);
            wave_layernorm256_rows<RW>(x1, lc, a.eps);
        }
        LAYER_DBG(19);
#pragma unroll
        for (int rr = 0; rr < RW; ++rr) {
            const int row = wave * RW + rr;
            if (q0 + row >= a.q_rows) x1[rr] = make_float4(0.f, 0.f, 0.f, 0.f);
            rows_to_h16(Xh, ldq, row, lane, x1[rr]);
        }
        LAYER_DBG(20);
    }
    __syncthreads();
    LAYER_DBG(6);
    unsigned short* Hh = R1;
    const int ldhh = 128 + HPAD;
    {
        f32x4 acc1[MTL][N1];
        acc_zero(acc1);
        gemm_packed<MTL, N1, PFF>(Xh, ldq, a.w1, 8, wave * N1, 8, 8, acc1, ring1);
        __syncthreads();
        acc_store_h16<MTL, N1>(acc1, Hh, ldhh, wave * (128 / WAVES), bias1, SEEME_ACT_GELU);
    }
    __syncthreads();
    LAYER_DBG(7);
    {
        f32x4 acc2[MTL][NTL];
        acc_zero(acc2);
        gemm_packed<MTL, NTL, PFW>(Hh, ldhh, a.w2, 4, wave * NTL, 16, 4, acc2, ring2);
        acc_store_lds<MTL, NTL>(acc2, Cs, ldc, wave * CW, bias2, SEEME_ACT_NONE);
    }
    const bool has_tail = a.skip_w != nullptr || a.qkv_w != nullptr || a.proj_w != nullptr;
    BRing<NTL, PFW> ring_t;
    if (a.skip_w != nullptr) prime_packed(ring_t, a.skip_w, 16, wave * NTL, 16, 8);
    else if (a.qkv_w != nullptr) prime_packed(ring_t, a.qkv_w, 8, wave * NTL, 48, 8);
    else if (a.proj_w != nullptr) prime_packed(ring_t, a.proj_w, 8, wave * NTL, (a.F + 15) >> 4, 8);
    __syncthreads();
    LAYER_DBG(8);
    {
        const LnParams lp = ln_params256_opt(a.n2_w, a.n2_b, a.n2_w), lf = ln_params256_opt(a.fin_w, a.fin_b, a.n2_w);
        float4 v[RW];
#pragma unroll
        for (int rr = 0; rr < RW; ++rr) {
            const float4 c = *reinterpret_cast<const float4*>(Cs + (wave * RW + rr) * ldc + lane * 4);
            v[rr] = make_float4(c.x + x1[rr].x, c.y + x1[rr].y, c.z + x1[rr].z, c.w + x1[rr].w);
        }
        wave_layernorm256_rows<RW>(v, lp, a.eps);
        if (a.fin_w != nullptr) wave_layernorm256_rows<RW>(v, lf, a.eps);
#pragma unroll
        for (int rr = 0; rr < RW; ++rr) {
            const int row = wave * RW + rr, s = q0 + row;
            if (s >= a.q_rows) v[rr] = make_float4(0.f, 0.f, 0.f, 0.f);
            if (a.out != nullptr && s < a.q_rows) {
                const size_t orow = a.out_mode == 1 ? (size_t)s * a.B + b : base + s;
                *reinterpret_cast<float4*>(a.out + orow * 256 + lane * 4) = v[rr];
            }
            if (has_tail) rows_to_h16(Xh, ldq, row, lane, v[rr]);
        }
    }
    LAYER_DBG(9);
    if (!has_tail) return;
    __syncthreads();
    if (a.skip_w != nullptr) {
        unsigned short* Sh = reinterpret_cast<unsigned short*>(R0);
        {
            float4 sv[RW];
#pragma unroll
            for (int rr = 0; rr < RW; ++rr) {
                const int s = q0 + wave * RW + rr;
                sv[rr] = *reinterpret_cast<const float4*>(a.skip_src + (base + (s < a.S ? s : 0)) * 256 + lane * 4);
                if (s >= a.S) sv[rr] = make_float4(0.f, 0.f, 0.f, 0.f);
            }
#pragma unroll
            for (int rr = 0; rr < RW; ++rr) rows_to_h16(Sh, ldq, wave * RW + rr, lane, sv[rr]);
        }
        const BiasRegs<NTL> bias_s = bias_load<NTL>(a.skip_b, wave * CW, 256);
        __syncthreads();
        f32x4 acc[MTL][NTL];
        acc_zero(acc);
        gemm_packed<MTL, NTL, PFW>(Xh, ldq, a.skip_w, 16, wave * NTL, 16, 8, acc, ring_t);
        gemm_packed<MTL, NTL, PFW>(Sh, ldq, a.skip_w + 8 * 64, 16, wave * NTL, 16, 8, acc);
        if (a.qkv_w != nullptr) prime_packed(ring_t, a.qkv_w, 8, wave * NTL, 48, 8);
        __syncthreads();
        acc_store_lds<MTL, NTL>(acc, Cs, ldc, wave * CW, bias_s, SEEME_ACT_NONE);
        __syncthreads();
#pragma unroll
        for (int rr = 0; rr < RW; ++rr) {
            const int row = wave * RW + rr, s = q0 + row;
            float4 v = *reinterpret_cast<const float4*>(Cs + row * ldc + lane * 4);
            if (s >= a.S) v = make_float4(0.f, 0.f, 0.f, 0.f);
            if (s < a.S) *reinterpret_cast<float4*>(a.xnext + (base + s) * 256 + lane * 4) = v;
            rows_to_h16(Xh, ldq, row, lane, v);
        }
        __syncthreads();
    }
    LAYER_DBG(10);
    if (a.qkv_w != nullptr) {
        tail_qkv_rows<WAVES, RW, PFW>(Xh, reinterpret_cast<unsigned short*>(R0), a.qkv_w, a.qkv_b, a.q_out, a.kp_out, a.vp_out, b, q0, a.S, a.spv, ring_t);
        LAYER_DBG(11);
        return;
    }
    if (a.proj_w != nullptr) {
        const int ntiles = (a.F + 15) >> 4;
        const BiasRegs<NTL> bias = bias_load<NTL>(a.proj_b, wave * CW, a.F);
        f32x4 acc[MTL][NTL];
        acc_zero(acc);
        if (wave * NTL < ntiles) gemm_packed<MTL, NTL, PFW>(Xh, ldq, a.proj_w, 8, wave * NTL, ntiles, 8, acc, ring_t);
        acc_store_lds<MTL, NTL>(acc, Cs, ldc, wave * CW, bias, SEEME_ACT_NONE);
        __syncthreads();
        for (int idx = tid; idx < ROWS * 256; idx += NT) {
            const int row = idx >> 8, c = idx & 255, s = q0 + row;
            if (s < a.S && c < a.F) a.feats[(base + s) * a.F + c] = Cs[row * ldc + c];
        }
    }
}

template <int WAVES, int RW>
static int launch_layer_w(const LayerHArgs& a, hipStream_t st) {
    constexpr int ROWS = RW * WAVES;
    if (a.z != nullptr && !layer_cvec_in<WAVES, RW>()) return seeme_fail("layer_h: this instantiation does not form the cross-attention vector");
    const size_t lds = (size_t)ROWS * (a.Sp + LDS_PAD) * 4 + (size_t)ROWS * (256 + HPAD) * 2 +
                       (layer_cvec_in<WAVES, RW>() ? (size_t)16 * (256 + HPAD) * 2 + 256 * 4 : 0);
    dim3 grid((a.q_rows + ROWS - 1) / ROWS, a.B);
    SEEME_HIP(hipFuncSetAttribute((const void*)k_layer_h<WAVES, RW>, hipFuncAttributeMaxDynamicSharedMemorySize, (int)lds));
    hipLaunchKernelGGL((k_layer_h<WAVES, RW>), grid, dim3(64 * WAVES), lds, st, a);
    return seeme_check_launch("k_layer_h");
}
static int layer_form(int B, int q_rows, int S) {
    static int rows = -1, w8_max = -1;
    if (rows < 0) { const char* e = getenv("SEEME_LAYER_ROWS"); rows = e ? atoi(e) : 32; }
    if (w8_max < 0) { const char* e = getenv("SEEME_LAYER_W8_MAX"); w8_max = e ? atoi(e) : 256; }
    const int Sp = (S + CH_N - 1) / CH_N * CH_N;
    if (rows == 64 && Sp <= 256 && q_rows > 32) return 2;
    const long wgs = (long)B * ((q_rows + 31) / 32);
    return wgs <= w8_max ? 1 : 0;
}
static bool layer_forms_cvec(int B, int q_rows, int S) { return layer_form(B, q_rows, S) == 1; }
static int launch_layer_h(const LayerHArgs& a_in, hipStream_t st) {
    LayerHArgs a = a_in;
    if (a.S <= 0 || a.S > 512) return seeme_fail("layer_h: S must be in 1..512");
    a.Sp = (a.S + CH_N - 1) / CH_N * CH_N;
    const int form = layer_form(a.B, a.q_rows, a.S);
    if (form == 2) return launch_layer_w<8, 8>(a, st);
    return form == 1 ? launch_layer_w<8, 4>(a, st) : launch_layer_w<4, 8>(a, st);
}


struct ProHArgs {
    int mode, B, S, T, F, spv;
    const float* features; const uint4* emb_w; const float* emb_b; const float* token; const float* pe;
    float* x;
    const uint4* qkv_w; const float* qkv_b; unsigned short* q_out; uint4* kp_out; uint4* vp_out;
};
__global__ __launch_bounds__(256) void k_vae_pro_h(const ProHArgs a) {
    extern __shared__ __attribute__((aligned(16))) float smem[];
    const int tid = threadIdx.x, wave = tid >> 6, lane = tid & 63;
    const int ldq = 256 + HPAD, ldc = 256 + LDS_PAD;
    float* Cs = smem;
    unsigned short* R1 = reinterpret_cast<unsigned short*>(Cs + TILE_M * ldc);
    const int b = blockIdx.y, q0 = blockIdx.x * TILE_M;
    const size_t base = (size_t)b * a.S;
    BRing<4, H16_PF> ring_t;
    if (a.mode == 1) {
        const int Kp = (a.F + 31) & ~31, lda_h = Kp + HPAD;
        const BiasRegs<4> bias = bias_load<4>(a.emb_b, wave * 64, 256);
        for (int idx = tid; idx < TILE_M * Kp; idx += 256) {
            const int row = idx / Kp, c = idx - row * Kp, s = q0 + row;
            const bool ok = s >= 2 && s < a.S && c < a.F;
            float v = a.features[ok ? ((size_t)b * a.T + (s - 2)) * a.F + c : 0];
            R1[row * lda_h + c] = f2h(ok ? v : 0.f);
        }
        __syncthreads();
        f32x4 acc[2][4];
        acc_zero(acc);
        gemm_packed<2, 4>(R1, lda_h, a.emb_w, Kp >> 5, wave * 4, 16, Kp >> 5, acc);
        acc_store_lds<2, 4>(acc, Cs, ldc, wave * 64, bias, SEEME_ACT_NONE);
    }
    prime_packed(ring_t, a.qkv_w, 8, wave * 4, 48, 8);
    __syncthreads();
    unsigned short* Xh = R1;
#pragma unroll
    for (int rr = 0; rr < 8; ++rr) {
        const int row = wave * 8 + rr, s = q0 + row, sc = s < a.S ? s : 0;
        float4 v = *reinterpret_cast<const float4*>(a.pe + (size_t)sc * 256 + lane * 4);
        if (a.mode == 1) {
            const float4 e = s < 2 ? *reinterpret_cast<const float4*>(a.token + (size_t)sc * 256 + lane * 4)
                                   : *reinterpret_cast<const float4*>(Cs + row * ldc + lane * 4);
            v = make_float4(v.x + e.x, v.y + e.y, v.z + e.z, v.w + e.w);
        }
        if (s >= a.S) v = make_float4(0.f, 0.f, 0.f, 0.f);
        else *reinterpret_cast<float4*>(a.x + (base + s) * 256 + lane * 4) = v;
        rows_to_h16(Xh, ldq, row, lane, v);
    }
    __syncthreads();
    tail_qkv_rows<4, 8, H16_PF>(Xh, reinterpret_cast<unsigned short*>(Cs), a.qkv_w, a.qkv_b, a.q_out, a.kp_out, a.vp_out, b, q0, a.S, a.spv, ring_t);
}
static int launch_pro_h(const ProHArgs& a, hipStream_t st) {
    if (a.mode == 1 && a.F > 256) return seeme_fail("vae_pro_h: nfeats > 256");
    const size_t lds = (size_t)TILE_M * (256 + LDS_PAD) * 4 + (size_t)TILE_M * (256 + HPAD) * 2;
    dim3 grid((a.S + TILE_M - 1) / TILE_M, a.B);
    SEEME_HIP(hipFuncSetAttribute((const void*)k_vae_pro_h, hipFuncAttributeMaxDynamicSharedMemorySize, (int)lds));
    hipLaunchKernelGGL(k_vae_pro_h, grid, dim3(256), lds, st, a);
    return seeme_check_launch("k_vae_pro_h");
}

__global__ void k_enc_tokens_h(const float* __restrict__ token, const float* __restrict__ pe, float* __restrict__ x, int B, int S) {
    const int idx = blockIdx.x * blockDim.x + threadIdx.x;
    if (idx >= B * 2 * 256) return;
    const int d = idx & 255, i = (idx >> 8) & 1, b = idx >> 9;
    x[((size_t)b * S + i) * 256 + d] = token[i * 256 + d] + pe[i * 256 + d];
}
__global__ void k_bcast_rows_h(const float* __restrict__ src, float* __restrict__ dst, int B, int rows) {
    const size_t idx = (size_t)blockIdx.x * blockDim.x + threadIdx.x;
    const size_t per = (size_t)rows * 64;
    if (idx >= per * B) return;
    reinterpret_cast<float4*>(dst)[idx] = reinterpret_cast<const float4*>(src)[idx % per];
}

struct WsH { float *x, *y, *sk0, *sk1, *cvec; unsigned short *qk, *vt; int spv; uint4* kp[2]; };
static WsH carve_h(void* ws, int B, int S) {
    const size_t R = (size_t)B * S;
    float* p = (float*)ws;
    WsH w;
    w.x = p; p += R * 256; w.y = p; p += R * 256; w.sk0 = p; p += R * 256; w.sk1 = p; p += R * 256;
    unsigned short* h = (unsigned short*)p;
    w.qk = h; h += R * 512;
    w.spv = (S + 31) & ~31;
    w.vt = h;
    p += R * 768;
    w.cvec = p;
    p += (size_t)B * 256 * (SEEME_NLAYERS + 1) + 64;
    w.kp[0] = reinterpret_cast<uint4*>(p);
    w.kp[1] = reinterpret_cast<uint4*>(reinterpret_cast<unsigned short*>(p) + (size_t)B * ((S + 15) & ~15) * 256);
    return w;
}

static int lin_h(hipStream_t st, const float* A, int lda, const uint16_t* wp, int K, int N, const float* bias, float* Y, int ldy,
                 int M, const float* pre_ln_w = nullptr, const float* pre_ln_b = nullptr) {
    LinearHArgs ha{};
    ha.k.a.A = A; ha.k.a.lda = lda; ha.k.a.K1 = K; ha.k.a.K = K; ha.k.a.bias = bias; ha.k.a.Y = Y; ha.k.a.ldy = ldy;
    ha.k.a.M = M; ha.k.a.N = N; ha.k.a.eps = 1e-5f; ha.k.a.pre_ln_w = pre_ln_w; ha.k.a.pre_ln_b = pre_ln_b;
    ha.wp = (const uint4*)wp; ha.kstride = ((K + 31) & ~31) >> 5; ha.ntiles = (N + 15) >> 4;
    return launch_linear_h(ha, st);
}

static int run_layer_h(hipStream_t st, const SeemeXfLayer& L, const SeemeXfLayerH& H, float* cur, float* mid, float* out, WsH& ws,
                       const int32_t* lengths, int B, int S, int n_prefix, int q_rows, const float* cvec, int cvec_ld,
                       const float* fin_w, const float* fin_b, int out_mode) {
    LinearHArgs q{};
    q.k.a.A = cur; q.k.a.lda = 256; q.k.a.K1 = 256; q.k.a.K = 256; q.k.a.bias = L.in_b; q.k.a.M = B * S; q.k.a.N = 768; q.k.a.eps = 1e-5f;
    q.wp = (const uint4*)H.in_w; q.kstride = 8; q.ntiles = 48; q.qkv_mode = 1; q.qk = ws.qk; q.vt = ws.vt; q.S = S; q.spv = ws.spv;
    int rc = ((reinterpret_cast<size_t>(cur) & 15) == 0) ? launch_qkv_h(q, st) : launch_linear_h(q, st);
    if (rc) return rc;
    AttnHArgs at{};
    at.qk = ws.qk; at.vt = ws.vt; at.res = cur; at.wo = (const uint4*)H.out_w; at.bo = L.out_b; at.ln_w = L.n1_w; at.ln_b = L.n1_b;
    at.out = mid; at.lengths = lengths; at.S = S; at.n_prefix = n_prefix; at.q_rows = q_rows; at.spv = ws.spv;
    at.scale = 1.0f / 16.0f; at.eps = 1e-5f;
    if ((rc = launch_attn_h(at, B, st))) return rc;
    FfnHArgs f{};
    f.x = mid; f.out = out; f.w1 = (const uint4*)H.l1_w; f.b1 = L.l1_b; f.w2 = (const uint4*)H.l2_w; f.b2 = L.l2_b;
    f.M = B * q_rows; f.FF = 128; f.act = SEEME_ACT_GELU; f.seq_rows = q_rows; f.seq_stride = S; f.out_mode = out_mode; f.eps = 1e-5f;
    f.fin_w = fin_w; f.fin_b = fin_b;
    if (cvec != nullptr) { f.cvec = cvec; f.cvec_ld = cvec_ld; f.lnc_w = L.n2_w; f.lnc_b = L.n2_b; f.ln_w = L.n3_w; f.ln_b = L.n3_b; }
    else { f.ln_w = L.n2_w; f.ln_b = L.n2_b; }
    return launch_ffn_h(f, st);
}

static int skip_lin_h(hipStream_t st, const float* a1, const float* a2, const uint16_t* wp, const float* b, float* y, int M) {
    LinearHArgs ha{};
    ha.k.a.A = a1; ha.k.a.lda = 256; ha.k.a.A2 = a2; ha.k.a.lda2 = 256; ha.k.a.K1 = 256; ha.k.a.K = 512; ha.k.a.bias = b;
    ha.k.a.Y = y; ha.k.a.ldy = 256; ha.k.a.M = M; ha.k.a.N = 256; ha.k.a.eps = 1e-5f;
    ha.wp = (const uint4*)wp; ha.kstride = 16; ha.ntiles = 16;
    return launch_linear_h(ha, st);
}

static void place_vt_unfused(WsH& ws, int S_carved) {
    if (ws.spv > 4 * S_carved) ws.vt = reinterpret_cast<unsigned short*>(ws.kp[0]);
}

static int vae_encode_h16_unfused(const SeemeVaeWeights* w, const float* features, const int32_t* lengths, int B, int T, float* mu,
                         void* workspace, hipStream_t st) {
    const SeemeVaeWeightsH* H = w->h16;
    const int S = T + 2, F = w->nfeats;
    WsH ws = carve_h(workspace, B, S);
    place_vt_unfused(ws, S);
    const SeemeSkipStack& E = w->enc;
    SEEME_HIP(hipMemsetAsync(ws.vt, 0, (size_t)B * 256 * ws.spv * 2, st));
    hipLaunchKernelGGL(k_enc_tokens_h, dim3((B * 512 + 255) / 256), dim3(256), 0, st, w->token, w->pe_enc, ws.x, B, S);
    int rc = seeme_check_launch("k_enc_tokens_h");
    if (rc) return rc;
    {
        LinearHArgs ha{};
        ha.k.a.A = features; ha.k.a.lda = F; ha.k.a.K1 = F; ha.k.a.K = F; ha.k.a.bias = w->emb_b; ha.k.a.res = w->pe_enc; ha.k.a.ldr = 256;
        ha.k.a.Y = ws.x; ha.k.a.ldy = 256; ha.k.a.M = B * T; ha.k.a.N = 256; ha.k.a.eps = 1e-5f;
        ha.k.seq_in = T; ha.k.in_stride = T; ha.k.out_stride = S; ha.k.out_off = 2; ha.k.res_mode = 1; ha.k.res_off = 2;
        ha.wp = (const uint4*)H->emb_w; ha.kstride = ((F + 31) & ~31) >> 5; ha.ntiles = 16;
        if ((rc = launch_linear_h(ha, st))) return rc;
    }
    if ((rc = run_layer_h(st, E.layer[0], H->enc[0], ws.x, ws.y, ws.sk0, ws, lengths, B, S, 2, S, nullptr, 0, nullptr, nullptr, 0))) return rc;
    if ((rc = run_layer_h(st, E.layer[1], H->enc[1], ws.sk0, ws.y, ws.sk1, ws, lengths, B, S, 2, S, nullptr, 0, nullptr, nullptr, 0))) return rc;
    if ((rc = run_layer_h(st, E.layer[2], H->enc[2], ws.sk1, ws.y, ws.x, ws, lengths, B, S, 2, S, nullptr, 0, nullptr, nullptr, 0))) return rc;
    if ((rc = skip_lin_h(st, ws.x, ws.sk1, H->enc_skip[0], E.skip_b[0], ws.x, B * S))) return rc;
    if ((rc = run_layer_h(st, E.layer[3], H->enc[3], ws.x, ws.y, ws.x, ws, lengths, B, S, 2, S, nullptr, 0, nullptr, nullptr, 0))) return rc;
    if ((rc = skip_lin_h(st, ws.x, ws.sk0, H->enc_skip[1], E.skip_b[1], ws.x, B * S))) return rc;
    return run_layer_h(st, E.layer[4], H->enc[4], ws.x, ws.y, mu, ws, lengths, B, S, 2, 2, nullptr, 0, E.norm_w, E.norm_b, 1);
}

static int vae_decode_h16_unfused(const SeemeVaeWeights* w, const float* z, const int32_t* lengths, int B, int T, float* feats,
                         void* workspace, hipStream_t st) {
    const SeemeVaeWeightsH* H = w->h16;
    const int S = T, F = w->nfeats;
    WsH ws = carve_h(workspace, B, S + 2);
    ws.spv = (S + 31) & ~31;
    place_vt_unfused(ws, S + 2);
    const SeemeSkipStack& Dk = w->dec;
    int rc;
    SEEME_HIP(hipMemsetAsync(ws.vt, 0, (size_t)B * 256 * ws.spv * 2, st));
    const int CL = SEEME_NLAYERS * 256;
    if ((rc = lin_h(st, z, 256, H->ca_fold_w, 256, CL, w->ca_fold_b, ws.cvec, CL, B))) return rc;
    {
        const size_t n4 = (size_t)B * S * 64;
        hipLaunchKernelGGL(k_bcast_rows_h, dim3((unsigned)((n4 + 255) / 256)), dim3(256), 0, st, w->pe_dec, ws.x, B, S);
        if ((rc = seeme_check_launch("k_bcast_rows_h"))) return rc;
    }
// ... 144 lines not shown
```

### seeme_amd/mld_denoiser.py

```python
from __future__ import annotations

import ctypes as C
import math
import os
from typing import Optional

import torch
import torch.nn as nn

from . import _lib as L
from .mld_vae import _PositionEmbeddingLearned1D, _EncoderLayerParams, _SkipStackParams, _param_fingerprint

_LAYER_FIELDS = ["skip", "inp", "outp", "l1", "l2", "caq", "cao", "f1", "f2", "fo",
                 "skip_b", "in_b", "out_b", "n1w", "n1b", "l1b", "l2b", "n2w", "n2b", "cnw", "cnb", "caq_b",
                 "csnw", "csnb", "cao_b", "f1b", "f2b", "fsnw", "fsnb", "fo_b"]


_CUS = {}


def _device_cus(device) -> int:
    idx = torch.device(device).index
    idx = torch.cuda.current_device() if idx is None else idx
    if idx not in _CUS:
        _CUS[idx] = int(torch.cuda.get_device_properties(idx).multi_processor_count)
    return _CUS[idx]


def timestep_features(timesteps: torch.Tensor, dim: int = 256, flip_sin_to_cos: bool = True,
                      freq_shift: float = 0.0, max_period: int = 10000) -> torch.Tensor:
    assert timesteps.dim() == 1
    half = dim // 2
    exponent = -math.log(max_period) * torch.arange(0, half, dtype=torch.float32, device=timesteps.device)
    exponent = exponent / (half - freq_shift)
    emb = timesteps[:, None].float() * torch.exp(exponent)[None, :]
    emb = torch.cat([torch.sin(emb), torch.cos(emb)], dim=-1)
    if flip_sin_to_cos:
        emb = torch.cat([emb[:, half:], emb[:, :half]], dim=-1)
    if dim % 2 == 1:
        emb = torch.nn.functional.pad(emb, (0, 1, 0, 0))
    return emb


def cluster_pack_stage(Wsub: torch.Tensor, TPW: int, KL: int, UL: int) -> torch.Tensor:
    EPL = KL // 4
    NT, K = Wsub.shape[0] // 16, Wsub.shape[1]
    assert NT == 8 * TPW and K % KL == 0 and (K // KL * TPW) % UL == 0
    KB = K // KL
    t = Wsub.reshape(NT, 16, KB, 4, EPL).permute(0, 2, 3, 1, 4).reshape(8, TPW, KB, 64, EPL)
    t = t.permute(0, 2, 1, 3, 4).reshape(8, (KB * TPW) // UL, UL, 64, EPL)
    return t.permute(1, 0, 2, 3, 4)


class _TimestepEmbeddingParams(nn.Module):
    def __init__(self, channel, time_embed_dim):
        super().__init__()
        self.linear_1 = nn.Linear(channel, time_embed_dim)
        self.linear_2 = nn.Linear(time_embed_dim, time_embed_dim)


class _StylizationParams(nn.Module):

    def __init__(self, d, t):
        super().__init__()
        self.emb_layers = nn.Sequential(nn.SiLU(), nn.Linear(t, 2 * d))
        self.norm = nn.LayerNorm(d)
        self.out_layers = nn.Sequential(nn.SiLU(), nn.Dropout(p=0.0), nn.Linear(d, d))


class _CrossAttnParams(nn.Module):
    def __init__(self, d, t):
        super().__init__()
        self.norm = nn.LayerNorm(d)
        self.text_norm = nn.LayerNorm(d)
        self.query = nn.Linear(d, d)
        self.key = nn.Linear(d, d)
        self.value = nn.Linear(d, d)
        self.proj_out = _StylizationParams(d, t)


class _FFNParams(nn.Module):
    def __init__(self, d, ff, t):
        super().__init__()
        self.linear1 = nn.Linear(d, ff)
        self.linear2 = nn.Linear(ff, d)
        self.proj_out = _StylizationParams(d, t)


class _MDLayerParams(nn.Module):

    def __init__(self, d, ff, nhead, dropout):
        super().__init__()
        self.d_model = d
        self.ca_block = _CrossAttnParams(d, d)
        self.ffn = _FFNParams(d, ff, d)
        self.sa_block = _EncoderLayerParams(d, nhead, 1024, dropout)


class MldDenoiser(nn.Module):

    def __init__(self,
                 ablation,
                 nfeats: int = 72,
                 condition: str = "text",
                 latent_dim: list = [1, 256],
                 ff_size: int = 128,
                 num_layers: int = 6,
                 num_heads: int = 4,
                 dropout: float = 0.1,
                 normalize_before: bool = False,
                 activation: str = "gelu",
                 flip_sin_to_cos: bool = True,
                 return_intermediate_dec: bool = False,
                 position_embedding: str = "learned",
                 arch: str = "trans_enc",
                 freq_shift: int = 0,
                 guidance_scale: float = 7.5,
                 guidance_uncondp: float = 0.1,
                 text_encoded_dim: int = 256,
                 nclasses: int = 10,
                 weight_dtype: str = "fp32",
                 cluster="auto",
                 **kwargs) -> None:
        super().__init__()
        self.latent_dim = latent_dim[-1]
        self.text_encoded_dim = text_encoded_dim
        self.condition = condition
        self.arch = arch
        self.pe_type = ablation.DIFF_PE_TYPE
        self.MD_trans = ablation.MD_TRANS
        self.flip_sin_to_cos, self.freq_shift = flip_sin_to_cos, freq_shift
        self.num_heads, self.ff_size, self.num_layers = num_heads, ff_size, num_layers
        if "text" not in self.condition:
            raise TypeError(f"condition type {self.condition} not supported")
        if self.pe_type != "mld":
            if self.pe_type == "actor":
                raise NotImplementedError("DIFF_PE_TYPE 'actor' is outside the accelerated path")
            raise ValueError("Not Support PE type")
        if arch != "trans_enc":
            if arch == "trans_dec":
                raise NotImplementedError("arch 'trans_dec' is outside the accelerated path")
            raise ValueError(f"Not supported architechure{self.arch}!")
        if ablation.VAE_TYPE == "no" or not ablation.SKIP_CONNECT or not self.MD_trans:
            raise NotImplementedError("accelerated path: VAE latent + SKIP_CONNECT + MD_TRANS (all SEE-ME configs)")
        if text_encoded_dim != self.latent_dim or self.latent_dim != 256 or latent_dim[0] != 1 or num_layers != 5:
            raise NotImplementedError("accelerated path: latent_dim [1,256], text_encoded_dim 256, 5 layers")
        if num_heads not in (1, 2, 4):
            raise NotImplementedError("accelerated path: num_heads in {1,2,4}")
        if weight_dtype not in ("fp32", "bf16", "fp16"):
            raise ValueError("weight_dtype must be 'fp32', 'bf16' or 'fp16'")
        self.weight_dtype = weight_dtype
        if cluster not in ("auto", 0, 2, 4, 8):
            raise ValueError("cluster must be 'auto', 0, 2, 4 or 8")
        self.cluster = cluster
        self.cluster_placement = 1
        self.cluster_flags = 0
        self.cluster_ms = True
        self.pack_xcds = "auto"

        d = self.latent_dim
        self.time_embedding = _TimestepEmbeddingParams(text_encoded_dim, d)
        self.query_pos = _PositionEmbeddingLearned1D(d)
        self.mem_pos = _PositionEmbeddingLearned1D(d)
        self.encoder = _SkipStackParams(lambda: _MDLayerParams(d, ff_size, num_heads, dropout), num_layers, d)

        self._wcache = None
        self._ws = L.Workspace(per_stream=False)
        self._table_cache = {}
        self._ccache = {}
        self._xchg = None

    def _layout(self):
        n = 5 * len(_LAYER_FIELDS) + 5
        buf = (C.c_int64 * n)()
        L.call("seeme_den_layout", 1024, self.ff_size, buf, n)
        vals = list(buf)
        layers = [dict(zip(_LAYER_FIELDS, vals[i * 30:(i + 1) * 30])) for i in range(5)]
        pe0, fnw, fnb, wg_total, vp_total = vals[150:155]
        self._layout_vals = vals
        return layers, pe0, fnw, fnb, wg_total, vp_total

    def _weights(self):
        fpnt = (_param_fingerprint(self), self.weight_dtype)
        if self._wcache is not None and self._wcache[0] == fpnt:
            return self._wcache[1]
        for p in self.parameters():
            L.require_cuda(p, "MldDenoiser parameter")
        dev = self.query_pos.pe.device
        layers, pe0, fnw, fnb, wg_total, vp_total = self._layout()
        bf16 = self.weight_dtype != "fp32"
        KV = 8 if bf16 else 4
        wdt = {"fp32": torch.float32, "bf16": torch.bfloat16, "fp16": torch.float16}[self.weight_dtype]
        wg = torch.zeros(wg_total, dtype=wdt, device=dev)
        vp = torch.zeros(vp_total, dtype=torch.float32, device=dev)

        def put_w(off, W):
            N, K = W.shape
            if bf16:
                TW, KB = N // 128, K // 32
                TG = 4 if TW % 4 == 0 else (3 if TW % 3 == 0 else (2 if TW % 2 == 0 else 1))
                g = W.detach().reshape(8, TW // TG, TG, 16, KB, 4, 8).permute(0, 1, 4, 2, 5, 3, 6).reshape(-1)
            else:
                g = W.detach().reshape(N, K // KV, KV).permute(1, 0, 2).reshape(-1)
            wg[off:off + g.numel()] = g.to(wg.dtype)

        def put_v(off, v):
            vp[off:off + v.numel()] = v.detach().reshape(-1)

        blocks = self.encoder.blocks()
        fold = self.num_heads == 1

        def sa_in_proj(sa):
            Wi, bi = sa.self_attn.in_proj_weight.detach(), sa.self_attn.in_proj_bias.detach()
            if not fold:
                return Wi, bi
            Wo, bo = sa.self_attn.out_proj.weight.detach().double(), sa.self_attn.out_proj.bias.detach().double()
            Wu = (Wo @ Wi[512:].double()).float()
            bu = (Wo @ bi[512:].double() + bo).float()
            return torch.cat([Wi[:512], Wu]), torch.cat([bi[:512], bu])

        with torch.no_grad():
            in_proj = [sa_in_proj(b.sa_block) for b in blocks]
            put_v(pe0, self.query_pos.pe[0, 0])
            put_v(fnw, self.encoder.norm.weight)
            put_v(fnb, self.encoder.norm.bias)
            for l, (blk, o) in enumerate(zip(blocks, layers)):
                sa, ca, ffn = blk.sa_block, blk.ca_block, blk.ffn
                if l >= 3:
                    put_w(o["skip"], self.encoder.linear_blocks[l - 3].weight)
                    put_v(o["skip_b"], self.encoder.linear_blocks[l - 3].bias)
                put_w(o["inp"], in_proj[l][0]); put_v(o["in_b"], in_proj[l][1])
                if not fold:
                    put_w(o["outp"], sa.self_attn.out_proj.weight); put_v(o["out_b"], sa.self_attn.out_proj.bias)
                put_w(o["l1"], sa.linear1.weight); put_v(o["l1b"], sa.linear1.bias)
                put_w(o["l2"], sa.linear2.weight); put_v(o["l2b"], sa.linear2.bias)
                put_v(o["n1w"], sa.norm1.weight); put_v(o["n1b"], sa.norm1.bias)
                put_v(o["n2w"], sa.norm2.weight); put_v(o["n2b"], sa.norm2.bias)
                put_v(o["cnw"], ca.norm.weight); put_v(o["cnb"], ca.norm.bias)
                put_w(o["caq"], ca.query.weight); put_v(o["caq_b"], ca.query.bias)
                put_v(o["csnw"], ca.proj_out.norm.weight); put_v(o["csnb"], ca.proj_out.norm.bias)
                put_w(o["cao"], ca.proj_out.out_layers[2].weight); put_v(o["cao_b"], ca.proj_out.out_layers[2].bias)
                put_w(o["f1"], ffn.linear1.weight); put_v(o["f1b"], ffn.linear1.bias)
                put_w(o["f2"], ffn.linear2.weight); put_v(o["f2b"], ffn.linear2.bias)
                put_v(o["fsnw"], ffn.proj_out.norm.weight); put_v(o["fsnb"], ffn.proj_out.norm.bias)
                put_w(o["fo"], ffn.proj_out.out_layers[2].weight); put_v(o["fo_b"], ffn.proj_out.out_layers[2].bias)
            kv_w = torch.cat([in_proj[l][0][256:] for l in range(len(blocks))]).contiguous()
            kv_b = torch.cat([in_proj[l][1][256:] for l in range(len(blocks))]).contiguous()
            st_w = torch.cat([torch.cat([b.ca_block.proj_out.emb_layers[1].weight, b.ffn.proj_out.emb_layers[1].weight])
                              for b in blocks]).contiguous()
            st_b = torch.cat([torch.cat([b.ca_block.proj_out.emb_layers[1].bias, b.ffn.proj_out.emb_layers[1].bias])
                              for b in blocks]).contiguous()
            ca_w = [torch.cat([b.ca_block.key.weight, b.ca_block.value.weight]).contiguous() for b in blocks]
            ca_b = [torch.cat([b.ca_block.key.bias, b.ca_block.value.bias]).contiguous() for b in blocks]
            cf_w = torch.cat([ca_w[l] * blk.ca_block.text_norm.weight[None, :] for l, blk in enumerate(blocks)]).contiguous()
            cf_b = torch.cat([ca_w[l] @ blk.ca_block.text_norm.bias + ca_b[l] for l, blk in enumerate(blocks)]).contiguous()
            ones, zeros = torch.ones(256, device=dev), torch.zeros(256, device=dev)
        lay_dev = torch.tensor(self._layout_vals, dtype=torch.int64, device=dev)
        w = L.DenoiserWeights()
        w.wg, w.wdtype, w.vp, w.layout = wg.data_ptr(), {"fp32": 0, "bf16": 1, "fp16": 2}[self.weight_dtype], vp.data_ptr(), lay_dev.data_ptr()
        w.nhead, w.ff_sa, w.ff = self.num_heads, 1024, self.ff_size
        w.kv_cat_w, w.kv_cat_b, w.style_cat_w, w.style_cat_b = kv_w.data_ptr(), kv_b.data_ptr(), st_w.data_ptr(), st_b.data_ptr()
        te = self.time_embedding
        w.time_w1, w.time_b1 = L.ptr(te.linear_1.weight), L.ptr(te.linear_1.bias)
        w.time_w2, w.time_b2 = L.ptr(te.linear_2.weight), L.ptr(te.linear_2.bias)
        for l, b in enumerate(blocks):
            w.ca_kv_w[l], w.ca_kv_b[l] = ca_w[l].data_ptr(), ca_b[l].data_ptr()
            w.ca_tn_w[l], w.ca_tn_b[l] = L.ptr(b.ca_block.text_norm.weight), L.ptr(b.ca_block.text_norm.bias)
        with torch.no_grad():
            pn_w = torch.stack([b.ca_block.proj_out.norm.weight for b in blocks]).contiguous()
            pn_b = torch.stack([b.ca_block.proj_out.norm.bias for b in blocks]).contiguous()
            po_w = torch.stack([b.ca_block.proj_out.out_layers[2].weight for b in blocks]).contiguous()
            po_b = torch.stack([b.ca_block.proj_out.out_layers[2].bias for b in blocks]).contiguous()
        w.ca_pn_w, w.ca_pn_b, w.ca_po_w, w.ca_po_b = pn_w.data_ptr(), pn_b.data_ptr(), po_w.data_ptr(), po_b.data_ptr()
        w.sa_fold = int(fold)
        w.ca_fold_w, w.ca_fold_b, w.ln_ones, w.ln_zeros = cf_w.data_ptr(), cf_b.data_ptr(), ones.data_ptr(), zeros.data_ptr()
        self._ccache = {}
        self._fold_parts = (in_proj, vp, layers)
        self._wcache = (fpnt, w, (wg, vp, kv_w, kv_b, st_w, st_b, ca_w, ca_b, lay_dev, cf_w, cf_b, ones, zeros, pn_w, pn_b, po_w, po_b))
        self._table_cache = {}
        return w

    def _cluster_weights(self, Cc: int, query: bool = False):
        self._weights()
        if (Cc, query) in self._ccache:
            return self._ccache[(Cc, query)]
        in_proj, vp, layers = self._fold_parts
        dev = vp.device
        code = {"fp32": 0, "bf16": 1, "fp16": 2}[self.weight_dtype]
        wdt = {"fp32": torch.float32, "bf16": torch.bfloat16, "fp16": torch.float16}[self.weight_dtype]
        lo = (C.c_int64 * 14)()
        L.call("seeme_den_cluster_layout", Cc, code, int(query), lo, 14)
        NU, UB, total, UL, KL = (int(v) for v in lo[:5])
        U_D, U_G, U_H = int(lo[9]), int(lo[12]), int(lo[13])
        EPL = KL // 4
        S, NB, TA, TB = 256 // Cc, 1024 // Cc, 256 // Cc // 32, 8 // Cc

        def pack_stage(Wsub, TPW):
            return cluster_pack_stage(Wsub, TPW, KL, UL)

        blocks = self.encoder.blocks()
        img = torch.zeros(5, Cc, NU, 8, UL, 64, EPL, dtype=wdt, device=dev)
        vpc = vp.clone()
        with torch.no_grad():
            for l, (blk, o) in enumerate(zip(blocks, layers)):
                Wq, bq = in_proj[l][0].double(), in_proj[l][1].double()
                if l >= 3:
                    Ws = self.encoder.linear_blocks[l - 3].weight.detach().double()
                    bs = self.encoder.linear_blocks[l - 3].bias.detach().double()
                    Wa = torch.cat([Wq @ Ws, Ws])
                    vpc[o["in_b"]:o["in_b"] + 768] = (Wq @ bs + bq).float()
                else:
                    Wa = torch.cat([Wq, torch.zeros(256, 256, dtype=torch.float64, device=dev)])
                W1, W2 = blk.sa_block.linear1.weight.detach(), blk.sa_block.linear2.weight.detach()
                Wf1, Wf2 = blk.ffn.linear1.weight.detach(), blk.ffn.linear2.weight.detach()
                Wfo = blk.ffn.proj_out.out_layers[2].weight.detach()
                for c in range(Cc):
                    rows = torch.cat([torch.arange(p * 256 + c * S, p * 256 + (c + 1) * S, device=dev) for p in range(4)])
                    ua = pack_stage(Wa[rows].to(wdt), TA)
                    img[l, c, 0:ua.shape[0]] = ua
                    img[l, c, 2 * TA:2 * TA + TB] = pack_stage(W1[c * NB:(c + 1) * NB].to(wdt), TB)
                    img[l, c, 2 * TA + TB:2 * TA + 2 * TB] = pack_stage(W2[:, c * NB:(c + 1) * NB].to(wdt), 2)
                    if query:
                        Wq_ca = blk.ca_block.query.weight.detach()[c * S:(c + 1) * S]
                        Wq_pad = torch.zeros(128, 256, dtype=Wq_ca.dtype, device=dev)
                        Wq_pad[:S] = Wq_ca
                        img[l, c, U_G:U_G + 1] = pack_stage(Wq_pad.to(wdt), 1)
                        img[l, c, U_H:U_H + 2] = pack_stage(blk.ca_block.proj_out.out_layers[2].weight.detach().to(wdt), 2)
                    u0 = U_D
                    img[l, c, u0:u0 + 1] = pack_stage(Wf1.to(wdt), 1)
                    img[l, c, u0 + 1:u0 + 2] = pack_stage(Wf2.to(wdt), 2)
                    img[l, c, u0 + 2:u0 + 4] = pack_stage(Wfo.to(wdt), 2)
        assert img.numel() * img.element_size() == total
        self._ccache[(Cc, query)] = (img, vpc, code)
        return self._ccache[(Cc, query)]

    def _cluster_size(self, B: int, N: int, cfg: bool, cus: int = 256) -> int:
        want = os.environ.get("SEEME_DEN_CLUSTER")
        want = self.cluster if want is None else (want if want == "auto" else int(want))
        if want == 0 or N > 2 or cfg or self.num_heads != 1:
            return 0
        Bp = (B + 7) // 8 * 8
        cus = min(int(cus), 256)
        if want == "auto":
            for Cc in (8, 4, 2):
                if Bp * Cc <= cus:
                    return Cc
            return 0
        return want if Bp * want <= cus else 0

    def _cluster_plan(self, B: int, N: int, cfg: bool, per_sample: bool, cus: int = 256):
        Cc = self._cluster_size(B, N, cfg, cus)
        want = os.environ.get("SEEME_DEN_CLUSTER")
        want = self.cluster if want is None else (want if want == "auto" else int(want))
        ms = os.environ.get("SEEME_DEN_CLUSTER_MS", "1") != "0" and self.cluster_ms
        forced = os.environ.get("SEEME_DEN_CLUSTER_MS_PLAN")
        if (want != "auto" or not ms or (B <= 32 and not forced) or N not in (1, 2) or cfg or per_sample or self.num_heads != 1
                or self.weight_dtype not in ("fp16", "bf16")):
            return Cc, 1
        if forced:
            C4, spc = (int(x) for x in forced.split(","))
            return C4, spc
        cus = min(int(cus), 256)
        if B <= 64 and Cc == 4:
            return Cc, 1
        ncl = (cus // 4) // 8 * 8
        most = 4 if self.weight_dtype == "bf16" else (8 if N == 1 else 6)
        if ncl >= 8 and -(-B // ncl) <= most:
            return 4, max(2, -(-B // ncl))
        return Cc, 1

    def cluster_status(self):
        if self._xchg is None:
            return (0, 0)
        hdr = self._xchg[:8].cpu().view(torch.int32)
        return int(hdr[0]), int(hdr[1])

    def _workspace(self, rows: int, device):
        return self._ws.get(L.lib().seeme_denoiser_workspace_bytes(rows, 0, 0), device)

    def time_tables(self, tfeat: torch.Tensor) -> torch.Tensor:
        L.require_cuda(tfeat, "tfeat")
        tfeat = tfeat.contiguous()
        rows = tfeat.shape[0]
        ttab = torch.empty(rows, L.TROW, device=tfeat.device, dtype=torch.float32)
        ws = self._workspace(rows, tfeat.device)
        w = self._weights()
        L.call("seeme_denoiser_time_tables", C.byref(w), tfeat.data_ptr(), rows, ttab.data_ptr(), ws.data_ptr(), ws.numel(),
               L.current_stream())
        return ttab

    def cond_tables(self, cond_bf: torch.Tensor) -> torch.Tensor:
        L.require_cuda(cond_bf, "condition")
        cond_bf = cond_bf.contiguous()
        Bc, N, _ = cond_bf.shape
        ctab = torch.empty(Bc, N, L.CROW, device=cond_bf.device, dtype=torch.float32)
        w = self._weights()
        L.call("seeme_denoiser_cond_tables", C.byref(w), cond_bf.data_ptr(), Bc, N, ctab.data_ptr(), 0, 0, L.current_stream())
        return ctab

    def ca_tables(self, ctab: torch.Tensor, ttab: torch.Tensor, trow: torch.Tensor, per_sample: bool) -> torch.Tensor:
        Bc = ctab.shape[0]
        R = 1 if per_sample else trow.numel()
        catab = torch.empty(Bc, R, 5, self.latent_dim, device=ctab.device, dtype=torch.float32)
        ws = torch.empty(5 * Bc * R * 256, device=ctab.device, dtype=torch.float32)
        w = self._weights()
        L.call("seeme_denoiser_ca_tables", C.byref(w), ctab.data_ptr(), ttab.data_ptr(), trow.data_ptr(), int(per_sample),
               trow.numel(), Bc, catab.data_ptr(), ws.data_ptr(), ws.numel() * 4, L.current_stream())
        return catab

    def _launch(self, latents2d, ctab, ttab, trow, per_sample, steps, sched, coef, noise, cfg, guidance):
        B, N = latents2d.shape[0], ctab.shape[1]
        out = torch.empty(B, self.latent_dim, device=latents2d.device, dtype=torch.float32)
        a = L.SampleArgs()
        a.B, a.N, a.steps, a.sched, a.cfg, a.guidance_scale = B, N, steps, sched, int(cfg), float(guidance)
        a.latents, a.ctab, a.ttab, a.trow, a.trow_per_sample = latents2d.data_ptr(), ctab.data_ptr(), ttab.data_ptr(), trow.data_ptr(), int(per_sample)
        a.coef, a.noise, a.out = L.ptr(coef), L.ptr(noise), out.data_ptr()
        catab = self.ca_tables(ctab, ttab, trow, per_sample) if N == 1 else None
        a.catab = L.ptr(catab)
        a.xcds = L.default_xcds((B + 1) // 2 if (B > 256 and not per_sample and not cfg) else B, self.pack_xcds)
        w = self._weights()
        Cc, spc = self._cluster_plan(B, N, bool(cfg), bool(per_sample), _device_cus(latents2d.device))
        if Cc:
            img, vpc, code = self._cluster_weights(Cc, N > 1)
            need = (L.lib().seeme_den_cluster_ms_xchg_bytes(B, Cc, spc) if spc > 1 else L.lib().seeme_den_cluster_xchg_bytes(B, Cc))
            if self._xchg is None or self._xchg.numel() < need or self._xchg.device != latents2d.device:
                self._xchg = torch.zeros(need, dtype=torch.uint8, device=latents2d.device)
            cl = L.DenCluster()
            cl.wgc, cl.wdtype, cl.vpc, cl.C = img.data_ptr(), code, vpc.data_ptr(), Cc
            cl.placement = int(os.environ.get("SEEME_DEN_CLUSTER_PLACE", self.cluster_placement))
            cl.flags = int(os.environ.get("SEEME_DEN_CLUSTER_FLAGS", self.cluster_flags))
            cl.xchg, cl.xchg_bytes = self._xchg.data_ptr(), self._xchg.numel()
            cl.query = int(N > 1)
            cl.samples = spc
            L.call("seeme_denoiser_sample_cluster", C.byref(w), C.byref(cl), C.byref(a), L.current_stream())
            return out
        L.call("seeme_denoiser_sample", C.byref(w), C.byref(a), L.current_stream())
        return out

    def forward(self, sample, timestep, encoder_hidden_states, lengths=None, **kwargs):
        L.require_cuda(sample, "sample")
        L.require_cuda(encoder_hidden_states, "encoder_hidden_states")
        B = sample.shape[0]
        if sample.shape[1] != 1:
            raise NotImplementedError("accelerated path: one latent token (latent_dim [1,256])")
        t = torch.as_tensor(timestep)
        per_sample = t.dim() > 0 and t.numel() > 1
        t1 = t.reshape(-1) if per_sample else t.reshape(1)
        tfeat = timestep_features(t1.to(sample.device), self.text_encoded_dim, self.flip_sin_to_cos, self.freq_shift)
        ttab = self.time_tables(tfeat.to(torch.float32))
        trow = (torch.arange(B, dtype=torch.int32, device=sample.device) if per_sample
                else torch.zeros(max(B, 1), dtype=torch.int32, device=sample.device))
        ctab = self.cond_tables(encoder_hidden_states.permute(1, 0, 2))
        out = self._launch(sample.reshape(B, -1).contiguous(), ctab, ttab, trow, True, 1, L.SCHED_NONE,
                           None, None, False, 1.0)
        return (out.reshape(B, 1, self.latent_dim),)

    def sample_loop(self, latents: torch.Tensor, cond_bf: torch.Tensor, scheduler, eta: float = 0.0,
                    guidance_scale: float = 1.0, step_noise: Optional[torch.Tensor] = None,
                    events=None) -> torch.Tensor:
        L.require_cuda(latents, "latents")
        B = latents.shape[0]
        cfg = guidance_scale > 1.0
        if cond_bf.shape[0] != (2 * B if cfg else B):
            raise ValueError("condition batch must be B (or 2B with classifier-free guidance)")
        dev = latents.device
        key = (tuple(scheduler.timesteps.tolist()), float(eta), type(scheduler).__name__)
        self._weights()
        cached = self._table_cache.get(key)
        if cached is None:
            tfeat = timestep_features(scheduler.timesteps.cpu(), self.text_encoded_dim, self.flip_sin_to_cos,
                                      self.freq_shift).to(dev)
            coef = scheduler.coef_table(eta).to(dev)
            trow = torch.arange(len(scheduler.timesteps), dtype=torch.int32, device=dev)
            cached = (tfeat, coef, trow, self.time_tables(tfeat))
            self._table_cache = {key: cached}
        tfeat, coef, trow, ttab = cached
        ctab = self.cond_tables(cond_bf)
        steps = len(trow)
        noise = None
        if scheduler.needs_noise(eta):
            if step_noise is None:
                step_noise = torch.randn(steps, B, self.latent_dim, device=dev, dtype=torch.float32)
            noise = step_noise.reshape(steps, B, self.latent_dim).contiguous()
        sched = L.SCHED_DDIM if type(scheduler).__name__.startswith("DDIM") else L.SCHED_DDPM
        lat2 = latents.reshape(B, -1).contiguous()
        if events is not None:
            events[0].record()
        out = self._launch(lat2, ctab, ttab, trow, False, steps, sched, coef, noise, cfg, guidance_scale)
        if events is not None:
            events[1].record()
        return out.reshape(1, B, self.latent_dim)
```

Baseline: 17650 seqs/s.

## Fuse condition and cross-attention table builds into one kernel with xchg zeroing

Adds a single k_den_tables1 kernel that computes the condition tables and the cross-attention tables together, and also zeroes the cluster exchange buffer. This replaces the separate cond_tables and ca_tables launches and the hipMemsetAsync before the cluster sampler. The change also vectorises the VAE prologue's feature staging using buffer loads. The aim is to cut launch count and small-kernel overhead in the per-call setup. In exchange the fused kernel is more complex, and the xchg zeroing now depends on the tables kernel having run first.

```diff
diff --git a/include/seeme_hip.h b/include/seeme_hip.h
--- a/include/seeme_hip.h
+++ b/include/seeme_hip.h
@@ -120,6 +120,10 @@
 int seeme_denoiser_ca_tables(const SeemeDenoiserWeights* w, const float* ctab, const float* ttab, const int32_t* trow,
                              int trow_per_sample, int n_trow, int Bc, float* catab,
                              void* workspace, size_t ws_bytes, void* stream);
+
+int seeme_denoiser_tables1(const SeemeDenoiserWeights* w, const float* cond, const float* ttab, const int32_t* trow,
+                           int trow_per_sample, int n_trow, int Bc, float* ctab, float* catab,
+                           void* zero, size_t zero_bytes, void* stream);
 
 typedef struct {
     int B;
@@ -156,6 +160,7 @@
     void* xchg; size_t xchg_bytes;
     int query;
     int samples;
+    int xchg_zeroed;
 } SeemeDenCluster;
 size_t seeme_den_cluster_xchg_bytes(int B, int C);
 size_t seeme_den_cluster_ms_xchg_bytes(int B, int C, int samples);
diff --git a/seeme_amd/_lib.py b/seeme_amd/_lib.py
--- a/seeme_amd/_lib.py
+++ b/seeme_amd/_lib.py
@@ -81,7 +81,8 @@
 
 class DenCluster(C.Structure):
     _fields_ = [("wgc", fp), ("wdtype", C.c_int), ("vpc", fp), ("C", C.c_int), ("placement", C.c_int), ("flags", C.c_int),
-                ("xchg", fp), ("xchg_bytes", C.c_size_t), ("query", C.c_int), ("samples", C.c_int)]
+                ("xchg", fp), ("xchg_bytes", C.c_size_t), ("query", C.c_int), ("samples", C.c_int),
+                ("xchg_zeroed", C.c_int)]
 
 
 class SmplModel(C.Structure):
@@ -197,6 +198,7 @@
     "seeme_denoiser_cond_tables": (C.c_int, [C.POINTER(DenoiserWeights), fp, C.c_int, C.c_int, fp, fp, C.c_size_t, fp]),
     "seeme_denoiser_ca_tables": (C.c_int, [C.POINTER(DenoiserWeights), fp, fp, fp, C.c_int, C.c_int, C.c_int, fp, fp, C.c_size_t, fp]),
     "seeme_denoiser_sample": (C.c_int, [C.POINTER(DenoiserWeights), C.POINTER(SampleArgs), fp]),
+    "seeme_denoiser_tables1": (C.c_int, [C.POINTER(DenoiserWeights), fp, fp, fp, C.c_int, C.c_int, C.c_int, fp, fp, fp, C.c_size_t, fp]),
     "seeme_denoiser_sample_cluster": (C.c_int, [C.POINTER(DenoiserWeights), C.POINTER(DenCluster), C.POINTER(SampleArgs), fp]),
     "seeme_den_cluster_xchg_bytes": (C.c_size_t, [C.c_int, C.c_int]),
     "seeme_den_cluster_ms_xchg_bytes": (C.c_size_t, [C.c_int, C.c_int, C.c_int]),
diff --git a/seeme_amd/csrc/den_cluster.inc.hip b/seeme_amd/csrc/den_cluster.inc.hip
--- a/seeme_amd/csrc/den_cluster.inc.hip
+++ b/seeme_amd/csrc/den_cluster.inc.hip
@@ -1111,7 +1111,7 @@
 }
 
 template <typename WT, int C, bool Q>
-static int launch_den_cluster(const ClArgs& ka0, hipStream_t st) {
+static int launch_den_cluster(const ClArgs& ka0, hipStream_t st, bool zeroed) {
     ClArgs ka = ka0;
     ka.clusters = (ka.s.B + 7) / 8 * 8;
     const int grid = ka.clusters * C;
@@ -1122,19 +1122,19 @@
     const size_t lds = cl_lds_bytes<C>(Q ? ka.s.N : 1, Q, ClGrp<WT, C, Q>::ON);
     if (lds > 160 * 1024 || lds <= 80 * 1024) return seeme_fail("denoiser_sample_cluster: LDS footprint must force one workgroup per CU");
     SEEME_HIP(hipFuncSetAttribute((const void*)k_den_cluster<WT, C, Q>, hipFuncAttributeMaxDynamicSharedMemorySize, (int)lds));
-    SEEME_HIP(hipMemsetAsync(ka.hdr, 0, seeme_den_cluster_xchg_bytes(ka.s.B, C), st));
+    if (!zeroed) SEEME_HIP(hipMemsetAsync(ka.hdr, 0, seeme_den_cluster_xchg_bytes(ka.s.B, C), st));
     hipLaunchKernelGGL((k_den_cluster<WT, C, Q>), dim3(grid), dim3(DEN_THREADS), lds, st, ka);
     return seeme_check_launch("k_den_cluster");
 }
 template <typename WT>
-static int launch_den_cluster_c(const ClArgs& ka, int C, bool q, hipStream_t st) {
-    if (C == 8) return q ? launch_den_cluster<WT, 8, true>(ka, st) : launch_den_cluster<WT, 8, false>(ka, st);
-    if (C == 4) return q ? launch_den_cluster<WT, 4, true>(ka, st) : launch_den_cluster<WT, 4, false>(ka, st);
-    if (C == 2) return q ? launch_den_cluster<WT, 2, true>(ka, st) : launch_den_cluster<WT, 2, false>(ka, st);
+static int launch_den_cluster_c(const ClArgs& ka, int C, bool q, hipStream_t st, bool zeroed) {
+    if (C == 8) return q ? launch_den_cluster<WT, 8, true>(ka, st, zeroed) : launch_den_cluster<WT, 8, false>(ka, st, zeroed);
+    if (C == 4) return q ? launch_den_cluster<WT, 4, true>(ka, st, zeroed) : launch_den_cluster<WT, 4, false>(ka, st, zeroed);
+    if (C == 2) return q ? launch_den_cluster<WT, 2, true>(ka, st, zeroed) : launch_den_cluster<WT, 2, false>(ka, st, zeroed);
     return seeme_fail("denoiser_sample_cluster: C must be 2, 4 or 8");
 }
 
-static int den_cluster_ms_dispatch(const SeemeDenoiserWeights* w, const SeemeDenCluster* cl, const SeemeSampleArgs* a, ClArgs& ka, hipStream_t st);
+static int den_cluster_ms_dispatch(const SeemeDenoiserWeights* w, const SeemeDenCluster* cl, const SeemeSampleArgs* a, ClArgs& ka, hipStream_t st, bool zeroed);
 
 extern "C" int seeme_denoiser_sample_cluster(const SeemeDenoiserWeights* w, const SeemeDenCluster* cl, const SeemeSampleArgs* a, void* stream) {
     if (a->B <= 0) return seeme_fail("denoiser_sample_cluster: B must be > 0");
@@ -1161,9 +1161,10 @@
     ka.xg = (unsigned long long*)((char*)cl->xchg + DCL_HDR_BYTES);
     ka.placement = cl->placement; ka.flags = cl->flags; ka.clusters = 0; ka.spc = 1;
     hipStream_t st = (hipStream_t)stream;
-    if (ms) return den_cluster_ms_dispatch(w, cl, a, ka, st);
-    if (cl->wdtype == 0) return launch_den_cluster_c<WF32>(ka, cl->C, q, st);
-    if (cl->wdtype == 1) return launch_den_cluster_c<WBF16>(ka, cl->C, q, st);
-    if (cl->wdtype == 2) return launch_den_cluster_c<WF16>(ka, cl->C, q, st);
+    const bool zeroed = cl->xchg_zeroed != 0;
+    if (ms) return den_cluster_ms_dispatch(w, cl, a, ka, st, zeroed);
+    if (cl->wdtype == 0) return launch_den_cluster_c<WF32>(ka, cl->C, q, st, zeroed);
+    if (cl->wdtype == 1) return launch_den_cluster_c<WBF16>(ka, cl->C, q, st, zeroed);
+    if (cl->wdtype == 2) return launch_den_cluster_c<WF16>(ka, cl->C, q, st, zeroed);
     return seeme_fail("denoiser_sample_cluster: wdtype must be 0 (fp32), 1 (bf16) or 2 (fp16)");
 }
diff --git a/seeme_amd/csrc/den_cluster_ms.inc.hip b/seeme_amd/csrc/den_cluster_ms.inc.hip
--- a/seeme_amd/csrc/den_cluster_ms.inc.hip
+++ b/seeme_amd/csrc/den_cluster_ms.inc.hip
@@ -732,7 +732,7 @@
 }
 
 template <typename WT, int C, bool Q, bool NARROW>
-static int launch_den_cluster_ms(const ClArgs& ka0, hipStream_t st) {
+static int launch_den_cluster_ms(const ClArgs& ka0, hipStream_t st, bool zeroed) {
     ClArgs ka = ka0;
     ka.clusters = clm_clusters(ka.s.B, ka.spc);
     const int grid = ka.clusters * C;
@@ -744,12 +744,12 @@
     const size_t lds = (size_t)ClM<WT, C, Q, NARROW>::LDS_FLOATS * sizeof(float);
     if (lds > 160 * 1024 || lds <= 80 * 1024) return seeme_fail("denoiser_sample_cluster: LDS footprint must force one workgroup per CU");
     SEEME_HIP(hipFuncSetAttribute((const void*)k_den_cluster_ms<WT, C, Q, NARROW>, hipFuncAttributeMaxDynamicSharedMemorySize, (int)lds));
-    SEEME_HIP(hipMemsetAsync(ka.hdr, 0, seeme_den_cluster_ms_xchg_bytes(ka.s.B, C, ka.spc), st));
+    if (!zeroed) SEEME_HIP(hipMemsetAsync(ka.hdr, 0, seeme_den_cluster_ms_xchg_bytes(ka.s.B, C, ka.spc), st));
     hipLaunchKernelGGL((k_den_cluster_ms<WT, C, Q, NARROW>), dim3(grid), dim3(DEN_THREADS), lds, st, ka);
     return seeme_check_launch("k_den_cluster_ms");
 }
 
-static int den_cluster_ms_dispatch(const SeemeDenoiserWeights* w, const SeemeDenCluster* cl, const SeemeSampleArgs* a, ClArgs& ka, hipStream_t st) {
+static int den_cluster_ms_dispatch(const SeemeDenoiserWeights* w, const SeemeDenCluster* cl, const SeemeSampleArgs* a, ClArgs& ka, hipStream_t st, bool zeroed) {
     if (cl->wdtype != 2 && cl->wdtype != 1) return seeme_fail("denoiser_sample_cluster: several samples per cluster need a 16-bit weight image");
     if (cl->C != 4 && cl->C != 8) return seeme_fail("denoiser_sample_cluster: several samples per cluster need C = 4 or 8");
     if (cl->samples > 8) return seeme_fail("denoiser_sample_cluster: at most 8 samples per cluster");
@@ -759,10 +759,10 @@
     ka.spc = cl->samples;
     if (cl->wdtype == 1) {
         if (cl->C != 4) return seeme_fail("denoiser_sample_cluster: the bf16 image takes several samples per cluster at C = 4 only");
-        return a->N == 2 ? launch_den_cluster_ms<WBF16, 4, true, false>(ka, st) : launch_den_cluster_ms<WBF16, 4, false, false>(ka, st);
+        return a->N == 2 ? launch_den_cluster_ms<WBF16, 4, true, false>(ka, st, zeroed) : launch_den_cluster_ms<WBF16, 4, false, false>(ka, st, zeroed);
     }
     if (cl->C == 4 && cl->samples <= 4)
-        return a->N == 2 ? launch_den_cluster_ms<WF16, 4, true, false>(ka, st) : launch_den_cluster_ms<WF16, 4, false, false>(ka, st);
-    if (a->N == 2) return cl->C == 8 ? launch_den_cluster_ms<WF16, 8, true, true>(ka, st) : launch_den_cluster_ms<WF16, 4, true, true>(ka, st);
-    return cl->C == 8 ? launch_den_cluster_ms<WF16, 8, false, true>(ka, st) : launch_den_cluster_ms<WF16, 4, false, true>(ka, st);
-}
+        return a->N == 2 ? launch_den_cluster_ms<WF16, 4, true, false>(ka, st, zeroed) : launch_den_cluster_ms<WF16, 4, false, false>(ka, st, zeroed);
+    if (a->N == 2) return cl->C == 8 ? launch_den_cluster_ms<WF16, 8, true, true>(ka, st, zeroed) : launch_den_cluster_ms<WF16, 4, true, true>(ka, st, zeroed);
+    return cl->C == 8 ? launch_den_cluster_ms<WF16, 8, false, true>(ka, st, zeroed) : launch_den_cluster_ms<WF16, 4, false, true>(ka, st, zeroed);
+}
diff --git a/seeme_amd/csrc/den_kernels.hip b/seeme_amd/csrc/den_kernels.hip
--- a/seeme_amd/csrc/den_kernels.hip
+++ b/seeme_amd/csrc/den_kernels.hip
@@ -966,6 +966,237 @@
     return seeme_launch_linear(ka, st);
 }
 
+struct Tables1Args {
+    const float* cond; const float* ttab; const int32_t* trow; int per_sample, n_trow, R, rows, Bc;
+    const float* kv_w; const float* kv_b; const float* cf_w; const float* cf_b; const float* ln_w; const float* ln_b;
+    const float* pn_w; const float* pn_b; const float* po_w; const float* po_b;
+    float* ctab; float* catab; unsigned char* zero; size_t zero_bytes;
+    int ca_blocks, ct_blocks, zero_blocks;
+};
+#define T1_LD (256 + LDS_PAD)
+__device__ __forceinline__ void t1_stage_cond(float* __restrict__ As, const float* __restrict__ cond, int b0, int n, bool ln,
+                                              const float* __restrict__ ln_w, const float* __restrict__ ln_b, int tid) {
+    const int wave = tid >> 6, lane = tid & 63;
+    const bool vec = (reinterpret_cast<size_t>(cond) & 15) == 0;
+    float lw[4], lb[4];
+#pragma unroll
+    for (int k = 0; k < 4; ++k) { lw[k] = ln_w[lane + 64 * k]; lb[k] = ln_b[lane + 64 * k]; }
+    float4 v[8];
+#pragma unroll
+    for (int j = 0; j < 8; ++j) {
+        const int row = 4 * j + wave;
+        const bool ok = row < n;
+        const float* p = ok ? cond + (size_t)(b0 + row) * 256 + 4 * lane : cond;
+        v[j] = vec ? ld4(p) : make_float4(p[0], p[1], p[2], p[3]);
+        if (!ok) v[j] = make_float4(0.f, 0.f, 0.f, 0.f);
+    }
+#pragma unroll
+    for (int j = 0; j < 8; ++j) st4(As + (4 * j + wave) * T1_LD + 4 * lane, v[j]);
+    __syncthreads();
+    if (ln) {
+        for (int rr = 0; rr < 8; ++rr) {
+            const int row = wave * 8 + rr;
+            if (row >= n) break;
+            float s = 0.f;
+            for (int c = lane; c < 256; c += 64) s += As[row * T1_LD + c];
+            const float mean = wave_sum(s) / 256.f;
+            float q = 0.f;
+            for (int c = lane; c < 256; c += 64) { float d = As[row * T1_LD + c] - mean; q += d * d; }
+            const float rs = 1.f / sqrtf(wave_sum(q) / 256.f + 1e-5f);
+#pragma unroll
+            for (int k = 0; k < 4; ++k) {
+                const int c = lane + 64 * k;
+                As[row * T1_LD + c] = (As[row * T1_LD + c] - mean) * rs * lw[k] + lb[k];
+            }
+        }
+        __syncthreads();
+    }
+}
+__device__ __forceinline__ float4 t1_ca_row(float4 v, float4 wv, float4 bv, float4 scl, float4 shf) {
+#pragma clang fp contract(off)
+    const float mean = wave_sum(v.x + v.y + v.z + v.w) * (1.f / 256.f);
+    const float4 c = make_float4(v.x - mean, v.y - mean, v.z - mean, v.w - mean);
+    const float xx = c.x * c.x, yy = c.y * c.y, zz = c.z * c.z, ww = c.w * c.w;
+    const float rs = fast_rsq(__builtin_fmaf(wave_sum(xx + yy + zz + ww), 1.f / 256.f, 1e-5f));
+    const float4 t = make_float4(c.x * rs, c.y * rs, c.z * rs, c.w * rs);
+    const float4 hn = make_float4(__builtin_fmaf(wv.x, t.x, bv.x), __builtin_fmaf(wv.y, t.y, bv.y), __builtin_fmaf(wv.z, t.z, bv.z), __builtin_fmaf(wv.w, t.w, bv.w));
+    const float4 one = make_float4(1.f + scl.x, 1.f + scl.y, 1.f + scl.z, 1.f + scl.w);
+    return f4_silu(make_float4(__builtin_fmaf(hn.x, one.x, shf.x), __builtin_fmaf(hn.y, one.y, shf.y), __builtin_fmaf(hn.z, one.z, shf.z), __builtin_fmaf(hn.w, one.w, shf.w)));
+}
+struct T1Ring { float4 br[4][4]; };
+__device__ __forceinline__ void t1_prime(T1Ring& R, const float* __restrict__ W, int n0) {
+    const int lane = threadIdx.x & 63, r = lane & 15, kq = lane >> 4;
+#pragma unroll
+    for (int u = 0; u < 4; ++u)
+#pragma unroll
+        for (int nt = 0; nt < 4; ++nt) R.br[u][nt] = ld4(W + ((unsigned)(n0 + nt * 16 + r) * 256u + 4u * kq + u * 16u));
+}
+template <int MTL>
+__device__ __forceinline__ void t1_gemm256(const float* __restrict__ As, const float* __restrict__ W, int n0, T1Ring& R, f32x4 (&acc)[MTL][4]) {
+    const int lane = threadIdx.x & 63, r = lane & 15, kq = lane >> 4;
+    unsigned wo[4];
+#pragma unroll
+    for (int nt = 0; nt < 4; ++nt) wo[nt] = (unsigned)(n0 + nt * 16 + r) * 256u + 4u * kq;
+    const float* ap = As + r * T1_LD + 4 * kq;
+#pragma unroll
+    for (int kb = 0; kb < 16; ++kb) {
+        const int u = kb & 3;
+        float4 av[MTL], b[4];
+#pragma unroll
+        for (int nt = 0; nt < 4; ++nt) b[nt] = R.br[u][nt];
+#pragma unroll
+        for (int mt = 0; mt < MTL; ++mt) av[mt] = ld4(ap + mt * 16 * T1_LD + kb * 16);
+        if (kb < 12) {
+#pragma unroll
+            for (int nt = 0; nt < 4; ++nt) R.br[u][nt] = ld4(W + (wo[nt] + (kb + 4) * 16u));
+        }
+        __builtin_amdgcn_sched_barrier(0);
+#pragma unroll
+        for (int mt = 0; mt < MTL; ++mt)
+#pragma unroll
+            for (int nt = 0; nt < 4; ++nt) acc[mt][nt] = __builtin_amdgcn_mfma_f32_16x16x4f32(av[mt].x, b[nt].x, acc[mt][nt], 0, 0, 0);
+#pragma unroll
+        for (int mt = 0; mt < MTL; ++mt)
+#pragma unroll
+            for (int nt = 0; nt < 4; ++nt) acc[mt][nt] = __builtin_amdgcn_mfma_f32_16x16x4f32(av[mt].y, b[nt].y, acc[mt][nt], 0, 0, 0);
+#pragma unroll
+        for (int mt = 0; mt < MTL; ++mt)
+#pragma unroll
+            for (int nt = 0; nt < 4; ++nt) acc[mt][nt] = __builtin_amdgcn_mfma_f32_16x16x4f32(av[mt].z, b[nt].z, acc[mt][nt], 0, 0, 0);
+#pragma unroll
+        for (int mt = 0; mt < MTL; ++mt)
+#pragma unroll
+            for (int nt = 0; nt < 4; ++nt) acc[mt][nt] = __builtin_amdgcn_mfma_f32_16x16x4f32(av[mt].w, b[nt].w, acc[mt][nt], 0, 0, 0);
+        __builtin_amdgcn_sched_barrier(0);
+    }
+}
+__device__ __forceinline__ void t1_store4(float* __restrict__ yp, float4 v, bool vec) {
+    if (vec) st4(yp, v);
+    else { yp[0] = v.x; yp[1] = v.y; yp[2] = v.z; yp[3] = v.w; }
+}
+__global__ __launch_bounds__(256, 2) void k_den_tables1(const Tables1Args a) {
+    extern __shared__ __attribute__((aligned(16))) float t1_smem[];
+    float* As = t1_smem;
+    float* Cs = t1_smem + TILE_M * T1_LD;
+    const int tid = threadIdx.x, wave = tid >> 6, lane = tid & 63;
+    int bid = blockIdx.x;
+    if (bid < a.ca_blocks) {
+        const int l = bid % SEEME_DEN_NL, m0 = (bid / SEEME_DEN_NL) * TILE_M;
+        const int mlast = m0 + TILE_M - 1 < a.rows ? m0 + TILE_M - 1 : a.rows - 1;
+        const int bc_lo = m0 / a.R, ns = mlast / a.R - bc_lo + 1;
+        const int ml = m0 + wave * 8 + (lane & 7), mlc = ml < a.rows ? ml : m0;
+        const int bcl = mlc / a.R, rl = mlc - bcl * a.R;
+        const int trl = a.trow[a.per_sample ? bcl % a.n_trow : rl];
+        const float* Wv = a.cf_w + (size_t)(l * 512 + 256) * 256;
+        const float* Wo = a.po_w + (size_t)l * 256 * 256;
+        T1Ring ring;
+        t1_prime(ring, Wv, wave * 64);
+        const BiasRegs<4> bias_v = bias_load<4>(a.cf_b + l * 512 + 256, wave * 64, 256);
+        const float4 pnw = ld4(a.pn_w + l * 256 + 4 * lane), pnb = ld4(a.pn_b + l * 256 + 4 * lane);
+        float4 tsc[8], tsh[8];
+        int srow[8];
+        const float* ttp[8];
+#pragma unroll
+        for (int rr = 0; rr < 8; ++rr) {
+            ttp[rr] = a.ttab + (size_t)__builtin_amdgcn_readlane(trl, rr) * SEEME_TROW + 2560 + l * 1024;
+            srow[rr] = __builtin_amdgcn_readlane(bcl, rr) - bc_lo;
+            if (rr < 4) { tsc[rr] = ld4(ttp[rr] + 4 * lane); tsh[rr] = ld4(ttp[rr] + 256 + 4 * lane); }
+        }
+        t1_stage_cond(As, a.cond, bc_lo, ns, true, a.ln_w, a.ln_b, tid);
+        if (ns <= 16) {
+            f32x4 acc[1][4];
+            acc_zero(acc);
+            t1_gemm256<1>(As, Wv, wave * 64, ring, acc);
+            acc_store_lds<1, 4>(acc, Cs, T1_LD, wave * 64, bias_v, SEEME_ACT_NONE);
+        } else {
+            f32x4 acc[2][4];
+            acc_zero(acc);
+            t1_gemm256<2>(As, Wv, wave * 64, ring, acc);
+            acc_store_lds<2, 4>(acc, Cs, T1_LD, wave * 64, bias_v, SEEME_ACT_NONE);
+        }
+#pragma unroll
+        for (int rr = 4; rr < 8; ++rr) { tsc[rr] = ld4(ttp[rr] + 4 * lane); tsh[rr] = ld4(ttp[rr] + 256 + 4 * lane); }
+        t1_prime(ring, Wo, wave * 64);
+        const BiasRegs<4> bias_o = bias_load<4>(a.po_b + l * 256, wave * 64, 256);
+        __syncthreads();
+#pragma unroll
+        for (int rr = 0; rr < 8; ++rr) {
+            const int row = wave * 8 + rr;
+            float4 o = t1_ca_row(ld4(Cs + srow[rr] * T1_LD + 4 * lane), pnw, pnb, tsc[rr], tsh[rr]);
+            if (m0 + row >= a.rows) o = make_float4(0.f, 0.f, 0.f, 0.f);
+            st4(As + row * T1_LD + 4 * lane, o);
+            if (rr == 3) __builtin_amdgcn_sched_barrier(0);
+        }
+        __syncthreads();
+        f32x4 acc[2][4];
+        acc_zero(acc);
+        t1_gemm256<2>(As, Wo, wave * 64, ring, acc);
+        acc_store_lds<2, 4>(acc, Cs, T1_LD, wave * 64, bias_o, SEEME_ACT_NONE);
+        __syncthreads();
+        const bool vec = (reinterpret_cast<size_t>(a.catab) & 15) == 0;
+#pragma unroll
+        for (int rr = 0; rr < 8; ++rr) {
+            const int row = wave * 8 + rr, m = m0 + row;
+            if (m >= a.rows) continue;
+            t1_store4(a.catab + ((size_t)m * SEEME_DEN_NL + l) * 256 + 4 * lane, ld4(Cs + row * T1_LD + 4 * lane), vec);
+        }
+        return;
+    }
+    bid -= a.ca_blocks;
+    if (bid < a.ct_blocks) {
+        const int by = bid % 40, z = (bid / 40) & 1, m0 = (bid / 80) * TILE_M, cn0 = by * 64;
+        const int n = a.Bc - m0 < TILE_M ? a.Bc - m0 : TILE_M;
+        t1_stage_cond(As, a.cond, m0, n, z == 1, a.ln_w, a.ln_b, tid);
+        f32x4 acc[2][1];
+        acc_zero(acc);
+        tile_gemm_f32<2, 1>(As, T1_LD, z ? a.cf_w : a.kv_w, 256, cn0 + wave * 16, 2560, 16, acc);
+        acc_store_lds<2, 1>(acc, Cs, T1_LD, wave * 16, z ? a.cf_b : a.kv_b, cn0, 2560, SEEME_ACT_NONE);
+        __syncthreads();
+        if (lane >= 16) return;
+        const bool vec = (reinterpret_cast<size_t>(a.ctab) & 15) == 0;
+#pragma unroll
+        for (int rr = 0; rr < 8; ++rr) {
+            const int row = wave * 8 + rr, m = m0 + row;
+            if (m >= a.Bc) continue;
+            t1_store4(a.ctab + (size_t)m * SEEME_CROW + z * 2560 + cn0 + 4 * lane, ld4(Cs + row * T1_LD + 4 * lane), vec);
+        }
+        return;
+    }
+    bid -= a.ct_blocks;
+    const size_t n16 = a.zero_bytes >> 4;
+    uint4* z16 = reinterpret_cast<uint4*>(a.zero);
+    for (size_t i = (size_t)bid * 256 + tid; i < n16; i += (size_t)a.zero_blocks * 256) z16[i] = make_uint4(0u, 0u, 0u, 0u);
+    if (bid == 0 && (size_t)tid < (a.zero_bytes & 15)) a.zero[(n16 << 4) + tid] = 0;
+}
+
+extern "C" int seeme_denoiser_tables1(const SeemeDenoiserWeights* w, const float* cond, const float* ttab, const int32_t* trow,
+                                      int trow_per_sample, int n_trow, int Bc, float* ctab, float* catab,
+                                      void* zero, size_t zero_bytes, void* stream) {
+    hipStream_t st = (hipStream_t)stream;
+    if (Bc <= 0 || n_trow <= 0) return seeme_fail("tables1: empty batch / row list");
+    if (w->ca_fold_w == nullptr) return seeme_fail("tables1: folded key/value weights missing");
+    if (w->ca_pn_w == nullptr || w->ca_po_w == nullptr) return seeme_fail("tables1: proj_out weights missing");
+    if (cond == nullptr || ttab == nullptr || trow == nullptr || ctab == nullptr || catab == nullptr) return seeme_fail("tables1: null table pointer");
+    if (zero_bytes != 0 && (zero == nullptr || ((uintptr_t)zero & 15) != 0)) return seeme_fail("tables1: the zero region must be 16-byte aligned");
+    Tables1Args a{};
+    a.cond = cond; a.ttab = ttab; a.trow = trow; a.per_sample = trow_per_sample; a.n_trow = n_trow;
+    a.R = trow_per_sample ? 1 : n_trow; a.Bc = Bc;
+    const long rows = (long)Bc * a.R;
+    if (rows > (1L << 30) / SEEME_DEN_NL) return seeme_fail("tables1: table too large");
+    a.rows = (int)rows;
+    a.kv_w = w->kv_cat_w; a.kv_b = w->kv_cat_b; a.cf_w = w->ca_fold_w; a.cf_b = w->ca_fold_b; a.ln_w = w->ln_ones; a.ln_b = w->ln_zeros;
+    a.pn_w = w->ca_pn_w; a.pn_b = w->ca_pn_b; a.po_w = w->ca_po_w; a.po_b = w->ca_po_b;
+    a.ctab = ctab; a.catab = catab; a.zero = (unsigned char*)zero; a.zero_bytes = zero_bytes;
+    a.ca_blocks = (a.rows + TILE_M - 1) / TILE_M * SEEME_DEN_NL;
+    a.ct_blocks = (Bc + TILE_M - 1) / TILE_M * 80;
+    const size_t zb = (zero_bytes + 256 * 16 * 4 - 1) / (256 * 16 * 4);
+    a.zero_blocks = (int)(zb < 64 ? zb : 64);
+    const size_t lds = (size_t)2 * TILE_M * T1_LD * sizeof(float);
+    SEEME_HIP(hipFuncSetAttribute((const void*)k_den_tables1, hipFuncAttributeMaxDynamicSharedMemorySize, (int)lds));
+    hipLaunchKernelGGL(k_den_tables1, dim3(a.ca_blocks + a.ct_blocks + a.zero_blocks), dim3(256), lds, st, a);
+    return seeme_check_launch("k_den_tables1");
+}
+
 #ifdef DEN_DBG_TIMES
 extern "C" int seeme_debug_den_times(unsigned long long* host, int n) {
     SEEME_HIP(hipMemcpyFromSymbol(host, HIP_SYMBOL(den_dbg_times), sizeof(unsigned long long) * (size_t)(n < 512 ? n : 512)));
diff --git a/seeme_amd/csrc/vae_h16.hip b/seeme_amd/csrc/vae_h16.hip
--- a/seeme_amd/csrc/vae_h16.hip
+++ b/seeme_amd/csrc/vae_h16.hip
@@ -1129,6 +1129,61 @@
     float* x;
     const uint4* qkv_w; const float* qkv_b; unsigned short* q_out; uint4* kp_out; uint4* vp_out;
 };
+template <int NB, bool VEC>
+__device__ __forceinline__ void pro_stage_features(const ProHArgs& a, unsigned short* __restrict__ R1, int lda_h, int b, int q0, int tid) {
+    const unsigned bytes = (unsigned)a.T * (unsigned)a.F * 4u;
+    const __amdgpu_buffer_rsrc_t rs = __builtin_amdgcn_make_buffer_rsrc(const_cast<float*>(a.features + (size_t)b * a.T * a.F), 0, (int)bytes, 0x00020000);
+    if (VEC) {
+        const int row = tid >> 3, sl = tid & 7, s = q0 + row;
+        const bool rok = s >= 2 && s < a.S;
+        const unsigned ro = (unsigned)(s - 2) * (unsigned)a.F * 4u;
+        float4 v[NB];
+#pragma unroll
+        for (int j = 0; j < NB; ++j) {
+            const int c = 4 * (sl + 8 * j);
+            const bool ok = rok && (j < NB - 1 || c < a.F);
+            v[j] = __builtin_bit_cast(float4, __builtin_amdgcn_raw_buffer_load_b128(rs, ok ? ro + 4u * c : bytes, 0, 0));
+        }
+#pragma unroll
+        for (int j = 0; j < NB; ++j) {
+            const unsigned lo = (unsigned)f2h(v[j].x) | ((unsigned)f2h(v[j].y) << 16), hi = (unsigned)f2h(v[j].z) | ((unsigned)f2h(v[j].w) << 16);
+            *reinterpret_cast<uint2*>(R1 + row * lda_h + 4 * (sl + 8 * j)) = make_uint2(lo, hi);
+        }
+    } else {
+        const int cl = tid & 31, rg = tid >> 5;
+        float v[4][NB];
+#pragma unroll
+        for (int i = 0; i < 4; ++i) {
+            const int s = q0 + rg + 8 * i;
+            const bool rok = s >= 2 && s < a.S;
+            const unsigned ro = (unsigned)(s - 2) * (unsigned)a.F * 4u;
+#pragma unroll
+            for (int j = 0; j < NB; ++j) {
+                const int c = cl + 32 * j;
+                const bool ok = rok && (j < NB - 1 || c < a.F);
+                v[i][j] = __builtin_bit_cast(float, __builtin_amdgcn_raw_buffer_load_b32(rs, ok ? ro + 4u * c : bytes, 0, 0));
+            }
+        }
+#pragma unroll
+        for (int i = 0; i < 4; ++i)
+#pragma unroll
+            for (int j = 0; j < NB; ++j) R1[(rg + 8 * i) * lda_h + cl + 32 * j] = f2h(v[i][j]);
+    }
+}
+template <bool VEC>
+__device__ __forceinline__ void pro_stage_features_nb(const ProHArgs& a, unsigned short* __restrict__ R1, int Kp, int b, int q0, int tid) {
+    const int lda_h = Kp + HPAD;
+    switch (Kp >> 5) {
+        case 1: pro_stage_features<1, VEC>(a, R1, lda_h, b, q0, tid); break;
+        case 2: pro_stage_features<2, VEC>(a, R1, lda_h, b, q0, tid); break;
+        case 3: pro_stage_features<3, VEC>(a, R1, lda_h, b, q0, tid); break;
+        case 4: pro_stage_features<4, VEC>(a, R1, lda_h, b, q0, tid); break;
+        case 5: pro_stage_features<5, VEC>(a, R1, lda_h, b, q0, tid); break;
+        case 6: pro_stage_features<6, VEC>(a, R1, lda_h, b, q0, tid); break;
+        case 7: pro_stage_features<7, VEC>(a, R1, lda_h, b, q0, tid); break;
+        default: pro_stage_features<8, VEC>(a, R1, lda_h, b, q0, tid); break;
+    }
+}
 __global__ __launch_bounds__(256) void k_vae_pro_h(const ProHArgs a) {
     extern __shared__ __attribute__((aligned(16))) float smem[];
     const int tid = threadIdx.x, wave = tid >> 6, lane = tid & 63;
@@ -1141,12 +1196,8 @@
     if (a.mode == 1) {
         const int Kp = (a.F + 31) & ~31, lda_h = Kp + HPAD;
         const BiasRegs<4> bias = bias_load<4>(a.emb_b, wave * 64, 256);
-        for (int idx = tid; idx < TILE_M * Kp; idx += 256) {
-            const int row = idx / Kp, c = idx - row * Kp, s = q0 + row;
-            const bool ok = s >= 2 && s < a.S && c < a.F;
-            float v = a.features[ok ? ((size_t)b * a.T + (s - 2)) * a.F + c : 0];
-            R1[row * lda_h + c] = f2h(ok ? v : 0.f);
-        }
+        if ((a.F & 3) == 0 && (reinterpret_cast<size_t>(a.features) & 15) == 0) pro_stage_features_nb<true>(a, R1, Kp, b, q0, tid);
+        else pro_stage_features_nb<false>(a, R1, Kp, b, q0, tid);
         __syncthreads();
         f32x4 acc[2][4];
         acc_zero(acc);
diff --git a/seeme_amd/mld_denoiser.py b/seeme_amd/mld_denoiser.py
--- a/seeme_amd/mld_denoiser.py
+++ b/seeme_amd/mld_denoiser.py
@@ -156,6 +156,7 @@
         self.cluster_placement = 1
         self.cluster_flags = 0
         self.cluster_ms = True
+        self.fused_tables = True
         self.pack_xcds = "auto"
 
         d = self.latent_dim
@@ -408,24 +409,52 @@
                trow.numel(), Bc, catab.data_ptr(), ws.data_ptr(), ws.numel() * 4, L.current_stream())
         return catab
 
-    def _launch(self, latents2d, ctab, ttab, trow, per_sample, steps, sched, coef, noise, cfg, guidance):
-        B, N = latents2d.shape[0], ctab.shape[1]
+    def _fused_tables(self) -> int:
+        e = os.environ.get("SEEME_DEN_TABLES")
+        return int(self.fused_tables) if e is None else int(e)
+
+    def tables1(self, cond_bf: torch.Tensor, ttab: torch.Tensor, trow: torch.Tensor, per_sample: bool, zero: Optional[torch.Tensor] = None,
+                zero_bytes: int = 0):
+        L.require_cuda(cond_bf, "condition")
+        cond_bf = cond_bf.contiguous()
+        Bc, N, _ = cond_bf.shape
+        if N != 1:
+            raise ValueError("tables1: one condition token")
+        R = 1 if per_sample else trow.numel()
+        ctab = torch.empty(Bc, 1, L.CROW, device=cond_bf.device, dtype=torch.float32)
+        catab = torch.empty(Bc, R, 5, self.latent_dim, device=cond_bf.device, dtype=torch.float32)
+        w = self._weights()
+        L.call("seeme_denoiser_tables1", C.byref(w), cond_bf.data_ptr(), ttab.data_ptr(), trow.data_ptr(), int(per_sample), trow.numel(), Bc,
+               ctab.data_ptr(), catab.data_ptr(), L.ptr(zero), int(zero_bytes) if zero is not None else 0, L.current_stream())
+        return ctab, catab
+
+    def _launch(self, latents2d, ctab, ttab, trow, per_sample, steps, sched, coef, noise, cfg, guidance, cond_bf=None):
+        fused = ctab is None
+        B, N = latents2d.shape[0], (1 if fused else ctab.shape[1])
         out = torch.empty(B, self.latent_dim, device=latents2d.device, dtype=torch.float32)
+        Cc, spc = self._cluster_plan(B, N, bool(cfg), bool(per_sample), _device_cus(latents2d.device))
+        need = 0
+        if Cc:
+            need = (L.lib().seeme_den_cluster_ms_xchg_bytes(B, Cc, spc) if spc > 1 else L.lib().seeme_den_cluster_xchg_bytes(B, Cc))
+            if self._xchg is None or self._xchg.numel() < need or self._xchg.device != latents2d.device:
+                self._xchg = torch.zeros(need, dtype=torch.uint8, device=latents2d.device)
+        catab = None
+        zeroed = fused and Cc and self._fused_tables() == 1
+        if fused:
+            ctab, catab = self.tables1(cond_bf, ttab, trow, per_sample, self._xchg if zeroed else None, need)
         a = L.SampleArgs()
         a.B, a.N, a.steps, a.sched, a.cfg, a.guidance_scale = B, N, steps, sched, int(cfg), float(guidance)
         a.latents, a.ctab, a.ttab, a.trow, a.trow_per_sample = latents2d.data_ptr(), ctab.data_ptr(), ttab.data_ptr(), trow.data_ptr(), int(per_sample)
         a.coef, a.noise, a.out = L.ptr(coef), L.ptr(noise), out.data_ptr()
-        catab = self.ca_tables(ctab, ttab, trow, per_sample) if N == 1 else None
+        if not fused and N == 1:
+            catab = self.ca_tables(ctab, ttab, trow, per_sample)
         a.catab = L.ptr(catab)
         a.xcds = L.default_xcds((B + 1) // 2 if (B > 256 and not per_sample and not cfg) else B, self.pack_xcds)
         w = self._weights()
-        Cc, spc = self._cluster_plan(B, N, bool(cfg), bool(per_sample), _device_cus(latents2d.device))
         if Cc:
             img, vpc, code = self._cluster_weights(Cc, N > 1)
-            need = (L.lib().seeme_den_cluster_ms_xchg_bytes(B, Cc, spc) if spc > 1 else L.lib().seeme_den_cluster_xchg_bytes(B, Cc))
-            if self._xchg is None or self._xchg.numel() < need or self._xchg.device != latents2d.device:
-                self._xchg = torch.zeros(need, dtype=torch.uint8, device=latents2d.device)
             cl = L.DenCluster()
+            cl.xchg_zeroed = int(bool(zeroed))
             cl.wgc, cl.wdtype, cl.vpc, cl.C = img.data_ptr(), code, vpc.data_ptr(), Cc
             cl.placement = int(os.environ.get("SEEME_DEN_CLUSTER_PLACE", self.cluster_placement))
             cl.flags = int(os.environ.get("SEEME_DEN_CLUSTER_FLAGS", self.cluster_flags))
@@ -475,7 +504,8 @@
             cached = (tfeat, coef, trow, self.time_tables(tfeat))
             self._table_cache = {key: cached}
         tfeat, coef, trow, ttab = cached
-        ctab = self.cond_tables(cond_bf)
+        fused = cond_bf.shape[1] == 1 and self._fused_tables() != 0
+        ctab = None if fused else self.cond_tables(cond_bf)
         steps = len(trow)
         noise = None
         if scheduler.needs_noise(eta):
@@ -486,7 +516,7 @@
         lat2 = latents.reshape(B, -1).contiguous()
         if events is not None:
             events[0].record()
-        out = self._launch(lat2, ctab, ttab, trow, False, steps, sched, coef, noise, cfg, guidance_scale)
+        out = self._launch(lat2, ctab, ttab, trow, False, steps, sched, coef, noise, cfg, guidance_scale, cond_bf=cond_bf)
         if events is not None:
             events[1].record()
         return out.reshape(1, B, self.latent_dim)
```

Result: faster. 17860 seqs/s (median of 6 runs) (+1.2%).
